# kakaobrain/hqtransformer

Hardware: NVIDIA B200
Metric: images_per_sec_sampled_256x256 (higher is better)
Workload: dtype bf16

## Files before the change

### hqtransformer_b200/_lib.py

```python
from __future__ import annotations

import ctypes as C
import os

PKG_DIR = os.path.dirname(os.path.abspath(__file__))
LIB_PATH = os.path.join(PKG_DIR, "libhqgraft.so")
ABI_VERSION = 8

HQ_OK = 0
HQ_COND_CLS, HQ_COND_TXT, HQ_COND_UNCOND = 0, 1, 2
HQ_PREC_BF16, HQ_PREC_FP32 = 0, 1
HQ_F32, HQ_BF16, HQ_F16 = 0, 1, 2
HQ_MODEL = {"parallel": 0, "top2bot": 1, "bidirectional": 2}
HQ_EMB = {"transformer1": 0, "reduce": 1}
HQ_POS = {"1d": 0, "2d": 1}


class HQConfig(C.Structure):
    _fields_ = [(n, C.c_int32) for n in (
        "embed_dim", "n_heads", "n_layers", "n_layers_depth", "vocab_top", "vocab_bot", "vocab_txt", "n_classes",
        "ctx_len_img", "ctx_len_txt", "cond_kind", "precision", "max_seq_len", "use_cuda_graph", "use_pdl", "use_chain", "model_type", "embedding_kind",
        "position_kind", "code_levels", "vocab_mid", "fuse_head_sampler")]


class HQSamplingParams(C.Structure):
    _fields_ = [("top_k_top", C.c_int32), ("top_k_bot", C.c_int32),
                ("top_p_top", C.c_float), ("top_p_bot", C.c_float),
                ("temperature_top", C.c_float), ("temperature_bot", C.c_float),
                ("seed", C.c_uint64), ("row_offset", C.c_uint64),
                ("top_k_mid", C.c_int32), ("top_p_mid", C.c_float), ("temperature_mid", C.c_float), ("reserved", C.c_int32)]


class HQRunArgs(C.Structure):
    _fields_ = [("batch", C.c_int32), ("seq_len", C.c_int32), ("pos_begin", C.c_int32), ("pos_end", C.c_int32),
                ("cond", C.c_void_p), ("sos", C.c_void_p), ("given_top", C.c_void_p), ("given_bot", C.c_void_p),
                ("codes_top", C.c_void_p), ("codes_bot", C.c_void_p), ("logits", C.c_void_p),
                ("sampling", HQSamplingParams), ("codes_mid", C.c_void_p), ("given_mid", C.c_void_p),
                ("shared_prefix", C.c_int32), ("reserved", C.c_int32)]


class HQS1Config(C.Structure):
    _fields_ = [("embed_dim", C.c_int32), ("n_embed", C.c_int32), ("z_channels", C.c_int32), ("resolution", C.c_int32),
                ("ch", C.c_int32), ("ch_mult", C.c_int32 * 8), ("n_levels", C.c_int32), ("num_res_blocks", C.c_int32),
                ("attn_resolution", C.c_int32), ("out_ch", C.c_int32)]


PROTOTYPES = {
    "hq_abi_version": (C.c_int, []),
    "hq_last_error": (C.c_char_p, [C.c_void_p]),
    "hq_create": (C.c_int, [C.POINTER(HQConfig), C.c_int, C.c_int, C.POINTER(C.c_void_p)]),
    "hq_destroy": (C.c_int, [C.c_void_p]),
    "hq_reserve_batch": (C.c_int, [C.c_void_p, C.c_int]),
    "hq_max_batch": (C.c_int, [C.c_void_p]),
    "hq_load_param": (C.c_int, [C.c_void_p, C.c_char_p, C.c_void_p, C.c_int, C.POINTER(C.c_int64), C.c_int, C.c_int]),
    "hq_params_complete": (C.c_int, [C.c_void_p]),
    "hq_run": (C.c_int, [C.c_void_p, C.POINTER(HQRunArgs), C.c_void_p]),
    "hq_run_host": (C.c_int, [C.c_void_p, C.POINTER(HQRunArgs)]),
    "hq_last_launch_count": (C.c_int64, [C.c_void_p]),
    "hq_device_bytes": (C.c_size_t, [C.c_void_p]),
    "hq_chain_launch_count": (C.c_int64, [C.c_void_p]),
    "hq_debug_gemm": (C.c_int, [C.c_int, C.c_void_p, C.c_void_p, C.c_void_p, C.c_int, C.c_int, C.c_int, C.c_int,
                             C.c_void_p]),
    "hq_debug_philox": (C.c_int, [C.c_uint64, C.POINTER(C.c_uint32), C.POINTER(C.c_uint32)]),
    "hq_debug_sample": (C.c_int, [C.c_void_p, C.c_int, C.c_int, C.c_float, C.c_int, C.c_float, C.c_uint64, C.c_uint64,
                                  C.c_int, C.c_int, C.c_void_p, C.c_void_p, C.c_void_p]),
    "hq_debug_attention": (C.c_int, [C.c_int, C.c_void_p, C.c_void_p, C.c_void_p, C.c_void_p, C.c_int, C.c_int, C.c_int,
                                     C.c_int, C.c_int, C.c_void_p]),
    "hq_debug_attention_phases": (C.c_int, [C.c_void_p, C.c_int, C.c_int, C.c_int, C.POINTER(C.c_uint64), C.c_int,
                                            C.POINTER(C.c_int), C.c_void_p]),
    "hq_debug_chain_phases": (C.c_int, [C.c_void_p, C.POINTER(HQRunArgs), C.c_void_p, C.c_int, C.c_int, C.POINTER(C.c_uint64),
                                        C.c_int, C.POINTER(C.c_int)]),
    "hq_bench_attention": (C.c_int, [C.c_void_p, C.c_int, C.c_int, C.c_int, C.POINTER(C.c_float), C.c_void_p]),
    "hq_trace_run": (C.c_int, [C.c_void_p, C.POINTER(HQRunArgs), C.c_void_p, C.POINTER(C.c_uint64), C.c_char_p, C.c_int,
                               C.POINTER(C.c_int)]),
    "hq_debug_gemm_phases": (C.c_int, [C.c_void_p, C.POINTER(HQRunArgs), C.c_void_p, C.c_int, C.POINTER(C.c_uint64), C.c_int,
                                       C.POINTER(C.c_uint64), C.c_char_p, C.c_int, C.POINTER(C.c_int)]),
    "hq_bench_gemm_shape": (C.c_int, [C.c_int, C.c_int, C.c_int, C.c_int, C.c_int, C.c_int, C.c_int, C.POINTER(C.c_float),
                                      C.POINTER(C.c_float), C.c_void_p]),
    "hq_bench_gemm": (C.c_int, [C.c_void_p, C.c_int, C.c_int, C.c_int, C.POINTER(C.c_float), C.c_void_p]),
    "hq_s1_create": (C.c_int, [C.POINTER(HQS1Config), C.c_int, C.c_int, C.POINTER(C.c_void_p)]),
    "hq_s1_destroy": (C.c_int, [C.c_void_p]),
    "hq_s1_last_error": (C.c_char_p, [C.c_void_p]),
    "hq_s1_device_bytes": (C.c_size_t, [C.c_void_p]),
    "hq_s1_load_param": (C.c_int, [C.c_void_p, C.c_char_p, C.c_void_p, C.c_int, C.POINTER(C.c_int64), C.c_int, C.c_int]),
    "hq_s1_params_complete": (C.c_int, [C.c_void_p]),
    "hq_s1_decode_codes": (C.c_int, [C.c_void_p, C.c_void_p, C.c_void_p, C.c_void_p, C.c_int, C.c_void_p]),
    "hq_s1_last_conv_flops": (C.c_double, [C.c_void_p]),
}

_lib = None


class HQError(RuntimeError):
    pass


def load() -> C.CDLL:
    global _lib
    if _lib is not None:
        return _lib
    if not os.path.isfile(LIB_PATH):
        raise ImportError(
            f"{LIB_PATH} is missing: build it with `python hqtransformer_b200/build.py` "
            "(hqtransformer_b200 has no CPU or PyTorch fallback path)")
    path = LIB_PATH
    if os.environ.get("HQ_DEBUG", "0") not in ("", "0") and os.environ.get("HQGRAFT_LIB"):
        path = os.environ["HQGRAFT_LIB"]
    lib = C.CDLL(path)
    for name, (res, args) in PROTOTYPES.items():
        fn = getattr(lib, name)
        fn.restype = res
        fn.argtypes = args
    got = lib.hq_abi_version()
    if got != ABI_VERSION:
        raise ImportError(f"libhqgraft.so ABI version {got} != binding version {ABI_VERSION}: rebuild the library")
    _lib = lib
    return lib


def check(rc: int, ctx=None, what: str = "") -> None:
    if rc != HQ_OK:
        msg = load().hq_last_error(ctx)
        raise HQError(f"{what or 'libhqgraft'} failed (status {rc}): {msg.decode() if msg else '?'}")


def check_s1(rc: int, ctx, lib, what: str = "") -> None:
    if rc != HQ_OK:
        msg = lib.hq_s1_last_error(ctx)
        raise HQError(f"{what or 'libhqgraft stage 1'} failed (status {rc}): {msg.decode() if msg else '?'}")
```

### hqtransformer_b200/csrc/engine.cu

```cuda
#include <cuda.h>
#include <cuda_runtime.h>

#include <cstdarg>
#include <cstdio>
#include <cstdlib>
#include <algorithm>
#include <cstring>
#include <map>
#include <string>
#include <tuple>
#include <vector>

#include "../../include/hqgraft.h"
#include "common.cuh"
#include "gemm.cuh"
#include "kernels.cuh"
#include "chain.cuh"

using namespace hq;

static thread_local std::string g_last_error;

struct hq_ctx;
static void set_err(hq_ctx* ctx, const char* fmt, ...);
// ... 63 lines not shown
  int bench_splits = 0;
  int force_bn = 0;
  int no_chain = 0;
  int chain_min_batch = 0;
  int chain_no_l2pf = 0;
  int gemm_ks1 = 0;
  int bn_m256 = 0;
};

static int env_int(const char* name) {
  const char* v = getenv(name);
  return v ? atoi(v) : 0;
}
static DebugSwitches read_debug_switches() {
  DebugSwitches d;
  const char* on = getenv("HQ_DEBUG");
  if (on == nullptr || atoi(on) == 0) return d;
  if (const char* a = getenv("HQ_ABLATE")) d.ablate = a;
  d.attn_groups = env_int("HQ_ATTN_GROUPS");
  d.attn_no_prefetch = getenv("HQ_ATTN_NO_PREFETCH") != nullptr;
  d.attn_sleep = env_int("HQ_ATTN_SLEEP");
  d.attn_scalar = getenv("HQ_ATTN_SCALAR") != nullptr;
  d.attm_stages = env_int("HQ_ATTM_STAGES");
  d.attm_per_sm = env_int("HQ_ATTM_PER_SM");
  d.attn_generic = getenv("HQ_ATTN_GENERIC") != nullptr;
  d.attn_fewkeys_old = getenv("HQ_ATTN_FEWKEYS_OLD") != nullptr;
  d.max_splitk = env_int("HQ_MAX_SPLITK");
  d.no_splitk = getenv("HQ_NO_SPLITK") != nullptr;
  d.force_splitk = env_int("HQ_FORCE_SPLITK");
  d.trace_pdl = getenv("HQ_TRACE_PDL") != nullptr;
  d.bench_splits = env_int("HQ_BENCH_SPLITS");
  d.no_chain = getenv("HQ_NO_CHAIN") != nullptr;
  d.chain_min_batch = env_int("HQ_CHAIN_MIN_BATCH");
  d.chain_no_l2pf = getenv("HQ_CHAIN_NO_L2PF") != nullptr;
  d.gemm_ks1 = getenv("HQ_GEMM_KS1") != nullptr;
  d.bn_m256 = env_int("HQ_BN_M256");
  return d;
}

struct GraphKey {
  int B, S, p0, p1, forced_top, forced_bot, sos_override, tracing;
  bool operator<(const GraphKey& o) const {
    return std::tie(B, S, p0, p1, forced_top, forced_bot, sos_override, tracing) <
           std::tie(o.B, o.S, o.p0, o.p1, o.forced_top, o.forced_bot, o.sos_override, o.tracing);
  }
};

struct hq_ctx {
  hq_config cfg;
  int device = 0, max_batch = 0;
  bool bf16 = true;
  int D = 0, nh = 0, L = 0, Ld = 0, Vt = 0, Vb = 0, Vmax = 0, T0 = 1, Tc = 0, Smax = 0;
  size_t wsize = 2;
  std::string err;
  std::vector<void*> allocs;
  std::vector<void*> act_allocs;
  bool alloc_act = false;
  size_t device_bytes = 0, act_bytes = 0;
  std::map<std::string, ParamSlot> params;
  PFN_encodeTiled encode = nullptr;

  std::vector<BlockW> blocks, depths;
  Weight head_top, head_bot;
  float *sos_table = nullptr, *sos_depth = nullptr;
  float *E_top = nullptr, *E_bot = nullptr, *P_emb = nullptr, *P_top = nullptr;
  float *E_txt = nullptr, *P_txt = nullptr;
  float *E_top_depth = nullptr, *P_depth = nullptr;
  float *E_bot_depth = nullptr;
  float *P_top_h = nullptr, *P_top_w = nullptr;
  int Hpos = 0;
  int depth_rows = 4;
  int levels = 2, n_stack = 5, Vm = 0;
  float *E_mid = nullptr, *E_mid_depth = nullptr, *P_depth2 = nullptr, *lnm_g = nullptr, *lnm_b = nullptr;
  Weight head_mid;
  int64_t* codes_mid = nullptr;
  float *lnf_g = nullptr, *lnf_b = nullptr, *lnt_g = nullptr, *lnt_b = nullptr, *lnb_g = nullptr, *lnb_b = nullptr;

  ABuf h, att, mlp;
  void* q = nullptr;
  float *x = nullptr, *yd = nullptr, *logits = nullptr;
  float2* samp_part = nullptr;
  float* splitk_ws = nullptr;
  unsigned int* att_sched = nullptr;
  CUtensorMap kmap, vmap;
  bool kv_maps = false;
  int num_sms = 0;
  int ws_rows = 0;
  void *kc = nullptr, *vc = nullptr, *kd = nullptr, *vd = nullptr;
  int64_t *cond = nullptr, *codes_top = nullptr, *codes_bot = nullptr;
  float* sos_override = nullptr;
  hq_sampling_params* d_sp = nullptr;

  cudaStream_t own_stream = nullptr;
  struct GraphEntry { cudaGraphExec_t exec; int64_t launches; uint64_t stamp; };
  static constexpr size_t kMaxGraphs = 96;
  std::map<GraphKey, GraphEntry> graphs;
  int64_t launches = 0;
  int64_t last_launches = 0;
  cudaError_t launch_err = cudaSuccess;
  bool use_pdl = false;
  bool tracing = false;
  int trace_cap = 0;
  std::vector<std::string> trace_tags;
  bool full_dependency_next = false;
  std::string tag_suffix;
  DebugSwitches dbg = read_debug_switches();
  uint64_t graph_clock = 0;

  bool chain_ok = false;
  int chain_grid = 0;
  CUtensorMap* d_maps = nullptr;
  ChainOp* d_ops = nullptr;
  int ops_cap = 0, ops_used = 0;
  std::map<std::string, int> chain_index;
  unsigned long long* d_chain_bar = nullptr;
  unsigned long long chain_epoch = 0;
  enum { CHAIN_OFF = 0, CHAIN_PLAN = 1, CHAIN_RUN = 2 };
  int chain_mode = CHAIN_OFF;
  bool recording = false;
  std::vector<ChainOp> rec;
  std::vector<std::string> rec_tags;
  int rec_flags = 0;
  const char* gemm_tag_override = nullptr;
  ChainRt chain_rt;
  std::vector<char> trace_chain_cont;
  int64_t chain_launches = 0, chain_ops = 0;
  int chain_launches_run = 0;
  int phase_launch = -1, phase_op = -1;
};

static void set_err(hq_ctx* ctx, const char* fmt, ...) {
  char buf[2048];
  va_list ap;
  va_start(ap, fmt);
  vsnprintf(buf, sizeof(buf), fmt, ap);
  va_end(ap);
  g_last_error = buf;
  if (ctx) ctx->err = buf;
}

static int dev_alloc(hq_ctx* ctx, void** p, size_t bytes) {
  bytes = (bytes + 255) & ~static_cast<size_t>(255);
  HQ_CUDA(ctx, cudaMalloc(p, bytes));
  HQ_CUDA(ctx, cudaMemset(*p, 0, bytes));
  if (ctx->alloc_act) {
    ctx->act_allocs.push_back(*p);
    ctx->act_bytes += bytes;
  } else {
    ctx->allocs.push_back(*p);
    ctx->device_bytes += bytes;
  }
  return HQ_OK;
}

static int make_map(hq_ctx* ctx, CUtensorMap* m, void* base, uint64_t rows, uint64_t cols, uint32_t box_rows) {
  cuuint64_t dims[2] = {cols, rows};
  cuuint64_t strides[1] = {cols * 2};
  cuuint32_t box[2] = {64, box_rows};
  cuuint32_t estr[2] = {1, 1};
  CUresult r = ctx->encode(m, CU_TENSOR_MAP_DATA_TYPE_BFLOAT16, 2, base, dims, strides, box, estr,
                           CU_TENSOR_MAP_INTERLEAVE_NONE, CU_TENSOR_MAP_SWIZZLE_128B, CU_TENSOR_MAP_L2_PROMOTION_L2_256B,
                           CU_TENSOR_MAP_FLOAT_OOB_FILL_NONE);
  if (r != CUDA_SUCCESS) {
    set_err(ctx, "cuTensorMapEncodeTiled failed (%d) rows=%llu cols=%llu", static_cast<int>(r),
            static_cast<unsigned long long>(rows), static_cast<unsigned long long>(cols));
    return HQ_ERR_CUDA;
  }
  return HQ_OK;
}

static int make_map3(hq_ctx* ctx, CUtensorMap* m, void* base, uint64_t rows, uint64_t cols, uint32_t box_rows, uint32_t ks) {
  cuuint64_t dims[3] = {64, rows, cols / 64};
  cuuint64_t strides[2] = {cols * 2, 128};
  cuuint32_t box[3] = {64, box_rows, ks};
  cuuint32_t estr[3] = {1, 1, 1};
  CUresult r = ctx->encode(m, CU_TENSOR_MAP_DATA_TYPE_BFLOAT16, 3, base, dims, strides, box, estr,
                           CU_TENSOR_MAP_INTERLEAVE_NONE, CU_TENSOR_MAP_SWIZZLE_128B, CU_TENSOR_MAP_L2_PROMOTION_L2_256B,
                           CU_TENSOR_MAP_FLOAT_OOB_FILL_NONE);
  if (r != CUDA_SUCCESS) {
    set_err(ctx, "cuTensorMapEncodeTiled (3-D k-block view) failed (%d) rows=%llu cols=%llu box_rows=%u", static_cast<int>(r),
            static_cast<unsigned long long>(rows), static_cast<unsigned long long>(cols), box_rows);
    return HQ_ERR_CUDA;
  }
  return HQ_OK;
}

static int make_pair_maps(hq_ctx* ctx, PairMaps* pm, void* base, uint64_t rows, uint64_t cols) {
  memset(pm, 0, sizeof(*pm));
  pm->have3 = cols >= 128;
  for (int i = 0; i < 6; ++i) {
    if (static_cast<uint64_t>(PairMaps::width(i)) > rows) continue;
    int rc = make_map(ctx, &pm->m[i], base, rows, cols, static_cast<uint32_t>(PairMaps::width(i) / 2));
    if (rc) return rc;
    if (pm->have3 && (rc = make_map3(ctx, &pm->m3[i], base, rows, cols, static_cast<uint32_t>(PairMaps::width(i) / 2), 2))) return rc;
  }
  return HQ_OK;
}

static int make_kv_map(hq_ctx* ctx, CUtensorMap* m, const void* base, int n_heads, uint64_t rows, int hpc) {
  cuuint64_t dims[3] = {64, static_cast<cuuint64_t>(n_heads), rows};
  cuuint64_t strides[2] = {128, static_cast<cuuint64_t>(n_heads) * 128};
  cuuint32_t box[3] = {64, static_cast<cuuint32_t>(hpc), 8};
  cuuint32_t estr[3] = {1, 1, 1};
  CUresult r = ctx->encode(m, CU_TENSOR_MAP_DATA_TYPE_BFLOAT16, 3, const_cast<void*>(base), dims, strides, box, estr,
                           CU_TENSOR_MAP_INTERLEAVE_NONE, CU_TENSOR_MAP_SWIZZLE_128B, CU_TENSOR_MAP_L2_PROMOTION_L2_256B,
                           CU_TENSOR_MAP_FLOAT_OOB_FILL_NONE);
  if (r != CUDA_SUCCESS) {
    set_err(ctx, "cuTensorMapEncodeTiled (KV cache) failed (%d) heads=%d rows=%llu hpc=%d", static_cast<int>(r), n_heads,
            static_cast<unsigned long long>(rows), hpc);
    return HQ_ERR_CUDA;
  }
  return HQ_OK;
}

static int alloc_weight(hq_ctx* ctx, Weight* w, int N, int K) {
  w->N = N;
  w->K = K;
  int rc = dev_alloc(ctx, &w->ptr, static_cast<size_t>(N) * K * ctx->wsize);
  if (rc) return rc;
  if (ctx->bf16) {
    if ((rc = make_map(ctx, &w->map, w->ptr, N, K, 64))) return rc;
    return make_pair_maps(ctx, &w->mapp, w->ptr, N, K);
  }
  return HQ_OK;
}
static int alloc_abuf(hq_ctx* ctx, ABuf* a, int rows, int K) {
  a->rows = (rows + 127) / 128 * 128;
  a->K = K;
  int rc = dev_alloc(ctx, &a->ptr, static_cast<size_t>(a->rows) * K * ctx->wsize);
  if (rc) return rc;
  if (ctx->bf16) {
    if ((rc = make_map(ctx, &a->map, a->ptr, a->rows, K, 128))) return rc;
    a->have3 = K >= 128;
    if (a->have3) return make_map3(ctx, &a->map3, a->ptr, a->rows, K, 128, 2);
  }
  return HQ_OK;
}
static int alloc_f32(hq_ctx* ctx, float** p, size_t n) { return dev_alloc(ctx, reinterpret_cast<void**>(p), n * 4); }

static void reg(hq_ctx* ctx, const std::string& name, void* dst, int is_weight, std::vector<int64_t> shape,
                bool ignored = false) {
  ParamSlot s;
  s.dst = dst;
  s.dst_is_weight = is_weight;
  s.shape = shape;
  s.ignored = ignored;
  ctx->params[name] = s;
}

static int build_block(hq_ctx* ctx, BlockW* b, const std::string& prefix) {
  const int D = ctx->D;
  int rc;
  if ((rc = alloc_weight(ctx, &b->qkv, 3 * D, D))) return rc;
  if ((rc = alloc_weight(ctx, &b->proj, D, D))) return rc;
  if ((rc = alloc_weight(ctx, &b->fc1, 4 * D, D))) return rc;
  if ((rc = alloc_weight(ctx, &b->fc2, D, 4 * D))) return rc;
  if ((rc = alloc_f32(ctx, &b->bqkv, 3 * D))) return rc;
  if ((rc = alloc_f32(ctx, &b->bproj, D))) return rc;
  if ((rc = alloc_f32(ctx, &b->b1, 4 * D))) return rc;
  if ((rc = alloc_f32(ctx, &b->b2, D))) return rc;
  float** lns[4] = {&b->ln1g, &b->ln1b, &b->ln2g, &b->ln2b};
  for (auto p : lns)
    if ((rc = alloc_f32(ctx, p, D))) return rc;
  const size_t wsz = ctx->wsize;
  char* wq = static_cast<char*>(b->qkv.ptr);
  reg(ctx, prefix + ".attn.query.weight", wq, 1, {D, D});
  reg(ctx, prefix + ".attn.key.weight", wq + static_cast<size_t>(D) * D * wsz, 1, {D, D});
  reg(ctx, prefix + ".attn.value.weight", wq + static_cast<size_t>(2) * D * D * wsz, 1, {D, D});
  reg(ctx, prefix + ".attn.query.bias", b->bqkv, 0, {D});
  reg(ctx, prefix + ".attn.key.bias", b->bqkv + D, 0, {D});
  reg(ctx, prefix + ".attn.value.bias", b->bqkv + 2 * D, 0, {D});
  reg(ctx, prefix + ".attn.proj.weight", b->proj.ptr, 1, {D, D});
  reg(ctx, prefix + ".attn.proj.bias", b->bproj, 0, {D});
  reg(ctx, prefix + ".mlp.0.weight", b->fc1.ptr, 1, {4 * D, D});
  reg(ctx, prefix + ".mlp.0.bias", b->b1, 0, {4 * D});
  reg(ctx, prefix + ".mlp.2.weight", b->fc2.ptr, 1, {D, 4 * D});
  reg(ctx, prefix + ".mlp.2.bias", b->b2, 0, {D});
  reg(ctx, prefix + ".ln1.weight", b->ln1g, 0, {D});
  reg(ctx, prefix + ".ln1.bias", b->ln1b, 0, {D});
  reg(ctx, prefix + ".ln2.weight", b->ln2g, 0, {D});
  reg(ctx, prefix + ".ln2.bias", b->ln2b, 0, {D});
  return HQ_OK;
}

template <typename K>
static int set_smem(hq_ctx* ctx, K kernel, int bytes) {
  HQ_CUDA(ctx, cudaFuncSetAttribute(kernel, cudaFuncAttributeMaxDynamicSharedMemorySize, bytes));
  return HQ_OK;
}

static int set_gemm_attrs(hq_ctx* ctx) {
  int rc;
#define HQ_SET(BN, EPI) \
// ... 61 lines not shown
extern "C" int hq_destroy(hq_ctx* ctx) {
  if (!ctx) return HQ_OK;
  cudaSetDevice(ctx->device);
  cudaDeviceSynchronize();
  free_activations(ctx);
  for (void* p : ctx->allocs) cudaFree(p);
  if (ctx->own_stream) cudaStreamDestroy(ctx->own_stream);
  delete ctx;
  return HQ_OK;
}

static void free_activations(hq_ctx* ctx) {
  for (auto& kv : ctx->graphs) cudaGraphExecDestroy(kv.second.exec);
  ctx->graphs.clear();
  for (void* p : ctx->act_allocs) cudaFree(p);
  ctx->act_allocs.clear();
  ctx->act_bytes = 0;
  ctx->d_maps = nullptr;
  ctx->chain_index.clear();
  ctx->ops_used = 0;
}

static int reserve_alloc(hq_ctx* ctx, int max_batch);

static int reserve_impl(hq_ctx* ctx, int max_batch) {
  const int rc = reserve_alloc(ctx, max_batch);
  if (rc != HQ_OK) {
    const std::string why = ctx->err;
    cudaGetLastError();
    free_activations(ctx);
    ctx->max_batch = 0;
    ctx->ws_rows = 0;
    ctx->kv_maps = false;
    ctx->h = ABuf(); ctx->att = ABuf(); ctx->mlp = ABuf();
    ctx->q = nullptr; ctx->x = nullptr; ctx->yd = nullptr; ctx->logits = nullptr; ctx->samp_part = nullptr; ctx->splitk_ws = nullptr;
    ctx->kc = ctx->vc = ctx->kd = ctx->vd = nullptr;
    ctx->cond = ctx->codes_top = ctx->codes_bot = ctx->codes_mid = nullptr;
    ctx->sos_override = nullptr;
    ctx->d_sp = nullptr;
    set_err(ctx, "hq_reserve_batch(%d) failed, the ctx holds no batch state until a reserve succeeds: %s", max_batch,
            why.c_str());
  }
  return rc;
}

static int reserve_alloc(hq_ctx* ctx, int max_batch) {
  int rc;
  if (max_batch < 1) {
    set_err(ctx, "max_batch must be >= 1");
    return HQ_ERR_INVALID;
  }
  HQ_CUDA(ctx, cudaSetDevice(ctx->device));
  HQ_CUDA(ctx, cudaDeviceSynchronize());
  free_activations(ctx);
  ctx->max_batch = max_batch;
  ctx->alloc_act = true;
  struct Guard { hq_ctx* c; ~Guard() { c->alloc_act = false; } } guard{ctx};
  const int D = ctx->D;
  const int B = max_batch;
  const int Mx = B * ctx->T0;
  const int Mmax = (ctx->depth_rows * B > Mx) ? ctx->depth_rows * B : Mx;
  if ((rc = alloc_abuf(ctx, &ctx->h, Mmax, D))) return rc;
  if ((rc = alloc_abuf(ctx, &ctx->att, Mmax, D))) return rc;
  if ((rc = alloc_abuf(ctx, &ctx->mlp, Mmax, 4 * D))) return rc;
  if ((rc = dev_alloc(ctx, &ctx->q, static_cast<size_t>(Mmax) * D * ctx->wsize))) return rc;
  if ((rc = alloc_f32(ctx, &ctx->x, static_cast<size_t>(Mx) * D))) return rc;
  if ((rc = alloc_f32(ctx, &ctx->yd, static_cast<size_t>(ctx->depth_rows) * B * D))) return rc;
  if ((rc = alloc_f32(ctx, &ctx->logits, static_cast<size_t>(ctx->depth_rows < 4 ? 4 : ctx->depth_rows) * B * ctx->Vmax))) return rc;
  {
    float* sp2 = nullptr;
    if ((rc = alloc_f32(ctx, &sp2, static_cast<size_t>(ctx->depth_rows < 4 ? 4 : ctx->depth_rows) * B * ((ctx->Vmax + 31) / 32) * 2))) return rc;
    ctx->samp_part = reinterpret_cast<float2*>(sp2);
  }
  ctx->ws_rows = Mmax;
  if (ctx->bf16 && (rc = alloc_f32(ctx, &ctx->splitk_ws, static_cast<size_t>(LN_MAXFOLD) * Mmax * D))) return rc;
  const size_t kvn = static_cast<size_t>(ctx->L) * B * ctx->Tc * D * ctx->wsize;
  if ((rc = dev_alloc(ctx, &ctx->kc, kvn))) return rc;
  if ((rc = dev_alloc(ctx, &ctx->vc, kvn))) return rc;
  ctx->kv_maps = false;
  if (ctx->bf16) {
    const int groups = attn_groups(ctx, ctx->nh);
    if (groups > 0) {
      const uint64_t rows = static_cast<uint64_t>(ctx->L) * B * ctx->Tc;
      if ((rc = make_kv_map(ctx, &ctx->kmap, ctx->kc, ctx->nh, rows, ctx->nh / groups))) return rc;
      if ((rc = make_kv_map(ctx, &ctx->vmap, ctx->vc, ctx->nh, rows, ctx->nh / groups))) return rc;
      ctx->kv_maps = true;
    }
  }
  const size_t kdn = static_cast<size_t>(ctx->Ld) * B * ctx->n_stack * D * ctx->wsize;
  if ((rc = dev_alloc(ctx, &ctx->kd, kdn))) return rc;
  if ((rc = dev_alloc(ctx, &ctx->vd, kdn))) return rc;
  if ((rc = dev_alloc(ctx, reinterpret_cast<void**>(&ctx->cond), static_cast<size_t>(B) * ctx->T0 * 8))) return rc;
  if ((rc = dev_alloc(ctx, reinterpret_cast<void**>(&ctx->codes_top), static_cast<size_t>(B) * ctx->Smax * 8))) return rc;
  if ((rc = dev_alloc(ctx, reinterpret_cast<void**>(&ctx->codes_bot),
                      static_cast<size_t>(B) * ctx->Smax * 8 * (ctx->levels == 3 ? 16 : 4)))) return rc;
  if (ctx->levels == 3 &&
      (rc = dev_alloc(ctx, reinterpret_cast<void**>(&ctx->codes_mid), static_cast<size_t>(B) * ctx->Smax * 32))) return rc;
  if ((rc = alloc_f32(ctx, &ctx->sos_override, static_cast<size_t>(Mx) * D))) return rc;
  if ((rc = dev_alloc(ctx, reinterpret_cast<void**>(&ctx->d_sp), sizeof(hq_sampling_params)))) return rc;
  if (ctx->bf16) {
    std::vector<CUtensorMap> table;
    ABuf* abufs[3] = {&ctx->h, &ctx->att, &ctx->mlp};
    for (ABuf* a : abufs) {
      a->map_idx = static_cast<int>(table.size());
      table.push_back(a->map);
    }
    auto add_w = [&](Weight& w) {
      w.map_idx = static_cast<int>(table.size());
      for (int i = 0; i < 6; ++i) table.push_back(w.mapp.m[i]);
    };
    for (auto& b : ctx->blocks) { add_w(b.qkv); add_w(b.proj); add_w(b.fc1); add_w(b.fc2); }
    for (auto& b : ctx->depths) { add_w(b.qkv); add_w(b.proj); add_w(b.fc1); add_w(b.fc2); }
    add_w(ctx->head_top);
    add_w(ctx->head_bot);
    if (ctx->levels == 3) add_w(ctx->head_mid);
    if ((rc = dev_alloc(ctx, reinterpret_cast<void**>(&ctx->d_maps), table.size() * sizeof(CUtensorMap)))) return rc;
    HQ_CUDA(ctx, cudaMemcpy(ctx->d_maps, table.data(), table.size() * sizeof(CUtensorMap), cudaMemcpyHostToDevice));
  }
  return HQ_OK;
}

static int create_impl(hq_ctx* ctx, const hq_config* cfg, int device, int max_batch) {
  int rc;
  if ((rc = check_device(ctx, device))) return rc;
  HQ_CUDA(ctx, cudaSetDevice(device));
  ctx->cfg = *cfg;
  ctx->device = device;
  ctx->max_batch = max_batch;
  ctx->bf16 = cfg->precision == HQ_PREC_BF16;
  ctx->use_pdl = cfg->use_pdl != 0;
  ctx->wsize = ctx->bf16 ? 2 : 4;
  const int D = ctx->D = cfg->embed_dim;
  ctx->nh = cfg->n_heads;
  ctx->L = cfg->n_layers;
  ctx->Ld = cfg->n_layers_depth;
  ctx->Vt = cfg->vocab_top;
  ctx->Vb = cfg->vocab_bot;
  ctx->Vmax = ctx->Vt > ctx->Vb ? ctx->Vt : ctx->Vb;
  ctx->levels = cfg->code_levels == 3 ? 3 : 2;
  if (cfg->code_levels != 0 && cfg->code_levels != 2 && cfg->code_levels != 3) {
    set_err(ctx, "code_levels must be 2 or 3 (got %d)", cfg->code_levels);
    return HQ_ERR_INVALID;
  }
  if (ctx->levels == 3) {
    ctx->Vm = cfg->vocab_mid;
    ctx->n_stack = 21;
    if (ctx->Vm > ctx->Vmax) ctx->Vmax = ctx->Vm;
    if (ctx->Vm < 64 || ctx->Vm % 64 != 0 || cfg->cond_kind == HQ_COND_TXT || cfg->model_type != HQ_MODEL_PARALLEL ||
        cfg->embedding_kind != HQ_EMB_TRANSFORMER1 || cfg->position_kind != HQ_POS_1D) {
      set_err(ctx, "code_levels == 3: the 'parallel-add' HQTransformer with class / unconditional sos, 'transformer1' embedding and "
                   "1-D positions is implemented (vocab_mid a multiple of 64)");
      return HQ_ERR_UNSUPPORTED;
    }
  }
  ctx->Smax = cfg->max_seq_len;
  const bool txt = cfg->cond_kind == HQ_COND_TXT;
  ctx->T0 = txt ? cfg->ctx_len_txt : 1;
  ctx->Tc = ctx->T0 + ctx->Smax - 1;
  if (max_batch < 1 || D < 64 || D % 64 != 0 || ctx->nh * 64 != D) {
    set_err(ctx, "unsupported shape: embed_dim=%d n_heads=%d (head size must be 64), max_batch=%d", D, ctx->nh, max_batch);
    return HQ_ERR_UNSUPPORTED;
  }
  if (ctx->Vt % 64 != 0 || ctx->Vb % 64 != 0 || ctx->Vmax > 32768) {
    set_err(ctx, "unsupported vocabulary sizes %d / %d (multiples of 64, <= 32768)", ctx->Vt, ctx->Vb);
    return HQ_ERR_UNSUPPORTED;
  }
  if (ctx->Tc > ATT_MAX_KEYS || ctx->Smax < 1 || ctx->Smax > cfg->ctx_len_img) {
    set_err(ctx, "unsupported lengths: max_seq_len=%d ctx_len_img=%d ctx_len_txt=%d (cache length %d > %d)", ctx->Smax,
// ... 505 lines not shown
  size_t stride = 0;
  const float* bias = nullptr;
};

template <typename AT>
static void layernorm_act(hq_ctx* ctx, cudaStream_t st, float* x, const float* g, const float* b, AT* out, int rows,
                          Fold* fold = nullptr) {
  Fold f = fold ? *fold : Fold();
  if (ctx->recording) {
    ChainOp* op = chain_push(ctx, CH_OP_LN, "layernorm");
    op->flags = sizeof(AT) == 4 ? CH_F_OUT_F32 : 0;
    op->x = x; op->gamma = g; op->beta = b; op->add = nullptr; op->out = out;
    op->rows = rows; op->in_mul = 1; op->in_off = 0; op->D = ctx->D;
    op->fold = f.partial; op->n_fold = f.n; op->fold_stride = f.stride; op->fold_bias = f.bias;
    if (fold) *fold = Fold();
    return;
  }
  auto kern = f.n > 3 ? layernorm_kernel<AT, LN_MAXFOLD> : layernorm_kernel<AT, 3>;
  launch_k(ctx, st, "layernorm", kern, dim3(rows), dim3(LN_THREADS), 0, x, g, b, nullptr, out, rows,
           ctx->D, 1, 0, f.partial, f.n, f.stride, f.bias, 1, 1);
  if (fold) *fold = Fold();
}

template <typename OutT>
static void layernorm_rows(hq_ctx* ctx, cudaStream_t st, const char* tag, float* x, const float* g, const float* b,
                           const float* add, OutT* out, int rows, int in_group, int in_mul, int in_off, int out_mul,
                           const Fold& f) {
  auto kern = f.n > 3 ? layernorm_kernel<OutT, LN_MAXFOLD> : layernorm_kernel<OutT, 3>;
  launch_k(ctx, st, tag, kern, dim3(rows), dim3(LN_THREADS), 0, x, g, b, add, out, rows, ctx->D, in_mul, in_off, f.partial,
           f.n, f.stride, f.bias, in_group, out_mul);
}

static bool attn_prefetch_ok(const hq_ctx* ctx) { return !ctx->dbg.attn_no_prefetch; }

static int attn_sleep_ns(const hq_ctx* ctx) { return ctx->dbg.attn_sleep; }

template <typename AT>
static bool attn_decode_plan(const hq_ctx* ctx, int* CH, int* hpc, int* groups, size_t* smem) {
  const int g = attn_groups(ctx, ctx->nh);
  if (g <= 0) return false;
  *groups = g;
  *hpc = ctx->nh / g;
  const int row_bytes = *hpc * 64 * static_cast<int>(sizeof(AT));
  int ch = (6144 / row_bytes) / 4 * 4;
  if (ch < 4) ch = 4;
  if (ch > 16) ch = 16;
  *CH = ch;
  *smem = static_cast<size_t>(ATTD_STAGES) * ch * row_bytes + static_cast<size_t>(*hpc) * ATT_MAX_KEYS * 4 +
          2 * ATTD_STAGES * 8 + 128;
  return *smem <= 64 * 1024;
}

static bool attn_mma_plan(const hq_ctx* ctx, int groups, int hpc, int n_items, int* stages, size_t* smem, int* grid) {
  if (ctx->dbg.attn_scalar || !ctx->bf16 || ctx->num_sms <= 0 || !ctx->kv_maps) return false;
  const size_t stage = static_cast<size_t>(2 * ATTM_CH) * hpc * 128;
  int st = 2;
  if (ctx->dbg.attm_stages) st = ctx->dbg.attm_stages;
  if (st < 2) st = 2;
  if (st > ATTM_MAXSTAGES) st = ATTM_MAXSTAGES;
  const size_t bytes = 1024  + st * stage + 2 * static_cast<size_t>(hpc) * 128 +
                       static_cast<size_t>(hpc) * 64 * 4 + (2 * ATTM_MAXSTAGES + 4) * 8 + 16;
  if (bytes > 112 * 1024) return false;
  int per_sm = static_cast<int>((227 * 1024) / (bytes + 1024));
  const int by_threads = 2048 / ((hpc + 1) * 32);
  if (per_sm > by_threads) per_sm = by_threads;
  const int by_regs = 65536 / ((hpc + 1) * 32 * 72);
  if (by_regs >= 1 && per_sm > by_regs) per_sm = by_regs;
  if (ctx->dbg.attm_per_sm > 0 && ctx->dbg.attm_per_sm < per_sm) per_sm = ctx->dbg.attm_per_sm;
  if (per_sm < 1) per_sm = 1;
  (void)groups;
  *stages = st;
  *smem = bytes;
  const int cap = ctx->num_sms * per_sm;
  *grid = n_items < cap ? n_items : cap;
  return true;
}

template <typename AT>
static void launch_attn_mma(hq_ctx*, cudaStream_t, const AT*, const AT*, AT*, int, int, int, int, int, int, int, size_t) {}
template <>
void launch_attn_mma<bf16>(hq_ctx* ctx, cudaStream_t st, const bf16* q, const bf16* K, bf16* out, int t_stride, int n_keys,
                           int hpc, int groups, int n_items, int stages, int grid, size_t smem) {
  const int row_base = static_cast<int>((K - static_cast<const bf16*>(ctx->kc)) / ctx->D);
  launch_k(ctx, st, "attention_decode", attention_decode_mma_kernel, dim3(grid), dim3((hpc + 1) * 32), smem, ctx->kmap, ctx->vmap,
           row_base, q, out, ctx->D, t_stride, n_keys, hpc, groups, n_items, attn_prefetch_ok(ctx) ? stages : -stages,
           ctx->att_sched);
}

template <typename AT>
static void attention(hq_ctx* ctx, cudaStream_t st, const AT* q, const AT* K, const AT* V, AT* out, int M, int Tq,
                      int t_stride, int kbase, int causal) {
  int CH = 0, hpc = 0, groups = 0;
  size_t smem = 0;
  if (ctx->recording && sizeof(AT) == 2 && !causal && kbase <= ATT_DEPTH_KEYS && Tq == 4) {
    ChainOp* op = chain_push(ctx, CH_OP_ATTN4, "attention_depth4");
    op->q = reinterpret_cast<const bf16*>(q); op->kc = reinterpret_cast<const bf16*>(K);
    op->vc = reinterpret_cast<const bf16*>(V); op->att = reinterpret_cast<bf16*>(out);
    op->B = M / 4; op->n_heads = ctx->nh; op->D = ctx->D; op->t_stride = t_stride; op->n_keys = kbase;
    return;
  }
  const bool resume = ctx->recording;
  if (resume) chain_flush(ctx, st);
  struct Resume { hq_ctx* c; bool on; ~Resume() { c->recording = on; } } resume_guard{ctx, resume};
  ctx->recording = false;
  if (Tq == 1 && !causal && !ctx->dbg.attn_generic && attn_decode_plan<AT>(ctx, &CH, &hpc, &groups, &smem)) {
    if (ctx->tracing) ctx->tag_suffix = ":t" + std::to_string(kbase) + ":B" + std::to_string(M);
    int stages = 0, grid = 0;
    size_t smem2 = 0;
    const ptrdiff_t koff = reinterpret_cast<const char*>(K) - static_cast<const char*>(ctx->kc);
    const ptrdiff_t kv_bytes = static_cast<ptrdiff_t>(ctx->L) * ctx->max_batch * ctx->Tc * ctx->D * static_cast<ptrdiff_t>(ctx->wsize);
    const bool in_cache = ctx->kc != nullptr && koff >= 0 && (koff < kv_bytes || ctx->L == 0) &&
                          koff == reinterpret_cast<const char*>(V) - static_cast<const char*>(ctx->vc);
    if (sizeof(AT) == 2 && in_cache && attn_mma_plan(ctx, groups, hpc, M * groups, &stages, &smem2, &grid)) {
      launch_attn_mma<AT>(ctx, st, q, K, out, t_stride, kbase, hpc, groups, M * groups, stages, grid, smem2);
      return;
    }
    launch_k(ctx, st, "attention_decode", attention_decode_kernel<AT>, dim3(M * groups), dim3((hpc + 1) * 32), smem, q, K, V,
             out, ctx->D, t_stride, kbase, CH, hpc, groups, attn_prefetch_ok(ctx) ? attn_sleep_ns(ctx) : -1);
    return;
  }
  const int items = M * ctx->nh;
  if (!causal && kbase <= ATT_DEPTH_KEYS && Tq == 4 && !ctx->dbg.attn_fewkeys_old) {
    const int warps = (M / 4) * ctx->nh;
    launch_k(ctx, st, "attention_depth4", attention_depth4_kernel<AT>, dim3((warps + ATT_WARPS - 1) / ATT_WARPS),
             dim3(ATT_WARPS * 32), 0, q, K, V, out, M / 4, ctx->nh, ctx->D, t_stride, kbase);
    return;
  }
  if (!causal && kbase <= 8) {
    launch_k(ctx, st, "attention_fewkeys", attention_fewkeys_kernel<AT>, dim3((items + ATT_WARPS - 1) / ATT_WARPS),
             dim3(ATT_WARPS * 32), 0, q, K, V, out, M, ctx->nh, ctx->D, Tq, t_stride, kbase);
    return;
  }
  launch_k(ctx, st, "attention_generic", attention_kernel<AT>, dim3((items + ATT_WARPS - 1) / ATT_WARPS),
           dim3(ATT_WARPS * 32), 0, q, K, V, out, M, ctx->nh, ctx->D, Tq, t_stride, kbase, causal);
}

static void launch_sample(hq_ctx* ctx, cudaStream_t st, const SampleArgs& a) {
  if (a.V <= 256 * SMP_IPT) launch_k(ctx, st, "sample", sample_kernel<256>, dim3(a.R), dim3(256), 0, a);
  else launch_k(ctx, st, "sample", sample_kernel<1024>, dim3(a.R), dim3(1024), 0, a);
}

static void gemm_fc2_split(hq_ctx* ctx, cudaStream_t st, const ABuf& A, const Weight& W, int M, int N, int K, int splits,
                           int bn, bf16*) {
  EpiParams<bf16> e;
  memset(&e, 0, sizeof(e));
  e.outf = ctx->splitk_ws; e.ldo = N; e.split_stride = static_cast<size_t>(ctx->ws_rows) * N;
  ctx->gemm_tag_override = "gemm_resid";
  gemm_bf16<EPI_F32>(ctx, st, A.map, A.have3 ? &A.map3 : nullptr, W.map, W.mapp, 0, M, N, K, e, splits, bn, A.map_idx, W.map_idx);
}
static void gemm_fc2_split(hq_ctx*, cudaStream_t, const ABuf&, const Weight&, int, int, int, int, int, float*) {}

struct Fc2Plan { int bn, splits; };

static int resid_splits(const hq_ctx* ctx, int N, int K, int rows_per_image) {
  static const int cand[6] = {256, 192, 128, 96, 64, 32};
  const int kb = K / 64;
  const int max_splits = ctx->dbg.max_splitk > 0 ? ctx->dbg.max_splitk : (kb % 3 == 0 ? 3 : LN_MAXFOLD);
  int best = 1;
  double best_cost = 1e30;
  for (int bn : cand) {
    if (N % bn != 0) continue;
    for (int s = 1; s <= max_splits && s <= LN_MAXFOLD; ++s) {
      if (kb % s != 0) continue;
      const double cost = pair_gemm_cost(256 * (rows_per_image < 1 ? 1 : rows_per_image), N, K, bn, s);
      if (cost < best_cost) {
        best_cost = cost;
        best = s;
      }
    }
  }
  return best;
}

static Fc2Plan pick_resid_plan(const hq_ctx* ctx, int M, int N, int K, int rows_per_image) {
  Fc2Plan best{0, 1};
  if (!ctx->bf16 || N % 64 != 0 || K % 64 != 0 || ctx->dbg.no_splitk) return best;
  static const int cand[6] = {256, 192, 128, 96, 64, 32};
  const int kb = K / 64;
  int s = resid_splits(ctx, N, K, rows_per_image);
  {
    const int v = ctx->dbg.force_splitk;
    if (v >= 1 && v <= LN_MAXFOLD && kb % v == 0) s = v;
  }
  best.splits = s;
  if (M <= 128) return best;
  double best_cost = 1e30;
  for (int bn : cand) {
    if (N % bn != 0) continue;
    const double cost = pair_gemm_cost(M, N, K, bn, s);
    if (cost < best_cost) {
      best_cost = cost;
      best.bn = bn;
    }
  }
  return best;
}

template <typename AT>
static void gemm_resid(hq_ctx* ctx, cudaStream_t st, const ABuf& A, const Weight& W, const float* bias, float* x, int M,
                       int N, int K, int rows_per_image, Fold* fold) {
  const Fc2Plan plan = pick_resid_plan(ctx, M, N, K, rows_per_image);
  if (plan.splits > 1 && M <= ctx->ws_rows) {
    gemm_fc2_split(ctx, st, A, W, M, N, K, plan.splits, plan.bn, static_cast<AT*>(nullptr));
    fold->partial = ctx->splitk_ws;
    fold->n = plan.splits;
    fold->stride = static_cast<size_t>(ctx->ws_rows) * N;
    fold->bias = bias;
    return;
  }
  EpiParams<AT> e;
  memset(&e, 0, sizeof(e));
  e.bias = bias; e.x = x;
  gemm_any<EPI_RESID>(ctx, st, A, W, 0, M, N, K, e);
}

template <typename AT>
static void run_block(hq_ctx* ctx, cudaStream_t st, const BlockW& w, float* x, int M, int mode, AT* kdst, AT* vdst,
                      int rpb, int t_stride, int t0, int n_keys_base, int causal, Fold* fold) {
  const int D = ctx->D;
  AT* h = static_cast<AT*>(ctx->h.ptr);
  AT* att = static_cast<AT*>(ctx->att.ptr);
  AT* mlp = static_cast<AT*>(ctx->mlp.ptr);
  AT* q = static_cast<AT*>(ctx->q);
  layernorm_act<AT>(ctx, st, x, w.ln1g, w.ln1b, h, M, fold);
  EpiParams<AT> ep;
  memset(&ep, 0, sizeof(ep));
  ep.q = q; ep.kdst = kdst; ep.vdst = vdst; ep.D = D; ep.rpb = rpb; ep.t_stride = t_stride; ep.t0 = t0;
  if (mode == 1) {
    ep.bias = w.bqkv + D; ep.sec0 = 1; ep.vdup = att;
    gemm_any<EPI_QKV>(ctx, st, ctx->h, w.qkv, D, M, 2 * D, D, ep);
  } else {
    ep.bias = w.bqkv; ep.sec0 = 0; ep.vdup = nullptr;
    if (mode == 0) ctx->rec_flags = CH_F_T0_RT;
    gemm_any<EPI_QKV>(ctx, st, ctx->h, w.qkv, 0, M, 3 * D, D, ep);
    ctx->rec_flags = 0;
    attention<AT>(ctx, st, q, kdst, vdst, att, M, rpb, t_stride, n_keys_base, causal);
  }
  gemm_resid<AT>(ctx, st, ctx->att, w.proj, w.bproj, x, M, D, D, rpb, fold);
  layernorm_act<AT>(ctx, st, x, w.ln2g, w.ln2b, h, M, fold);
  EpiParams<AT> eg;
  memset(&eg, 0, sizeof(eg));
  eg.bias = w.b1; eg.out = mlp;
  gemm_any<EPI_GELU>(ctx, st, ctx->h, w.fc1, 0, M, 4 * D, D, eg);
  gemm_resid<AT>(ctx, st, ctx->mlp, w.fc2, w.b2, x, M, D, 4 * D, rpb, fold);
}

struct RunFlags {
  int forced_top, forced_bot, sos_override, forced_mid;
  int shared_prefix;
  int fuse_mask;
  float* logits_out;
};

template <typename AT>
static bool head_gemm(hq_ctx* ctx, cudaStream_t st, const Weight& w, int rows, int V, const SampleArgs& sa, const RunFlags& f) {
  const bool fuse = sizeof(AT) == 2 && !ctx->recording && ((f.fuse_mask >> sa.filt_sel) & 1) && !sa.forced &&
                    sa.logits_out == nullptr && V % 32 == 0;
  EpiParams<AT> e;
  memset(&e, 0, sizeof(e));
  if (fuse) {
    e.sp = sa.sp; e.samp_part = ctx->samp_part; e.temp_sel = sa.temp_sel; e.rows_per_b = sa.rows_per_b; e.slot0 = sa.slot0;
    e.pos = sa.pos;
    ctx->gemm_tag_override = "gemm_head_sample";
    gemm_any<EPI_SAMPLE>(ctx, st, ctx->h, w, 0, rows, V, ctx->D, e);
  } else {
    e.outf = ctx->logits; e.ldo = ctx->Vmax;
    gemm_any<EPI_F32>(ctx, st, ctx->h, w, 0, rows, V, ctx->D, e);
  }
  return fuse;
}

static void draw(hq_ctx* ctx, cudaStream_t st, const SampleArgs& sa, bool fused) {
  if (fused)
    launch_k(ctx, st, "sample_finalize", sample_finalize_kernel, dim3((sa.R + SMPF_WARPS - 1) / SMPF_WARPS), dim3(SMPF_WARPS * 32),
             0, sa, static_cast<const float2*>(ctx->samp_part), sa.V / 32);
  else if (!(sa.forced && sa.logits_out == nullptr))
    launch_sample(ctx, st, sa);
}

template <typename AT>
static void run_position(hq_ctx* ctx, cudaStream_t st, int B, int S, int pos, const RunFlags& f) {
  const int D = ctx->D, T0 = ctx->T0, Tc = ctx->Tc;
  const bool txt = ctx->cfg.cond_kind == HQ_COND_TXT;
  const bool prefill = txt && pos == 0;
  const bool shared = prefill && f.shared_prefix && B > 1;
  const int Bp = shared ? 1 : B;
  const int M = prefill ? Bp * T0 : B;
  AT* kc = static_cast<AT*>(ctx->kc);
  AT* vc = static_cast<AT*>(ctx->vc);
  AT* kd = static_cast<AT*>(ctx->kd);
  AT* vd = static_cast<AT*>(ctx->vd);
  AT* h = static_cast<AT*>(ctx->h.ptr);
  const size_t lstride = static_cast<size_t>(ctx->max_batch) * Tc * D;
  const size_t dstride = static_cast<size_t>(ctx->max_batch) * 5 * D;

  const int eb = (D / 4 + 31) / 32 * 32 > 1024 ? 1024 : (D / 4 + 31) / 32 * 32;
  Fold fold_x, fold_y;
  ctx->full_dependency_next = true;
  if (prefill) {
    launch_k(ctx, st, "embed_txt", embed_txt_kernel, dim3(M), dim3(eb), 0, ctx->x, f.sos_override ? ctx->sos_override : nullptr,
             ctx->cond, ctx->E_txt, ctx->P_txt, T0, D);
  } else {
    EmbedArgs ea;
    ea.x = ctx->x; ea.sos_table = ctx->sos_table; ea.sos_override = f.sos_override ? ctx->sos_override : nullptr;
    ea.cond = ctx->cond; ea.E_top = ctx->E_top; ea.E_bot = ctx->E_bot; ea.P_top = ctx->P_top; ea.P_emb = ctx->P_emb;
    ea.codes_top = ctx->codes_top; ea.codes_bot = ctx->codes_bot; ea.D = D; ea.S = S; ea.pos = pos;
    ea.cond_kind = ctx->cfg.cond_kind;
    ea.emb_kind = ctx->cfg.embedding_kind; ea.P_top_h = ctx->P_top_h; ea.P_top_w = ctx->P_top_w; ea.Hpos = ctx->Hpos;
    launch_k(ctx, st, "embed", embed_kernel, dim3(B), dim3(eb), 0, ea);
  }

  const int tok = (pos == 0) ? 0 : T0 + pos - 1;
  const bool chain = sizeof(AT) == 2 && !prefill && chain_enabled(ctx, B);
  if (chain) chain_begin(ctx, tok, pos, S);
  for (int l = 0; l < ctx->L; ++l) {
    if (prefill) run_block<AT>(ctx, st, ctx->blocks[l], ctx->x, M, 0, kc + l * lstride, vc + l * lstride, T0, Tc, 0, 0, 1, &fold_x);
    else run_block<AT>(ctx, st, ctx->blocks[l], ctx->x, M, 0, kc + l * lstride, vc + l * lstride, 1, Tc, tok, tok + 1, 0, &fold_x);
  }
  if (ctx->recording) {
    ChainOp* op = chain_push(ctx, CH_OP_LN, "layernorm_f");
    op->flags = CH_F_OUT_F32;
    op->x = ctx->x; op->gamma = ctx->lnf_g; op->beta = ctx->lnf_b; op->add = ctx->sos_depth; op->out = ctx->yd;
    op->rows = B; op->in_mul = 1; op->in_off = 0; op->D = D;
    op->fold = fold_x.partial; op->n_fold = fold_x.n; op->fold_stride = fold_x.stride; op->fold_bias = fold_x.bias;
  } else {
    launch_k(ctx, st, "layernorm_f", fold_x.n > 3 ? layernorm_kernel<float, LN_MAXFOLD> : layernorm_kernel<float, 3>, dim3(B),
             dim3(LN_THREADS), 0, ctx->x, ctx->lnf_g, ctx->lnf_b,
             ctx->sos_depth, ctx->yd, prefill ? Bp : B, D, prefill ? T0 : 1, prefill ? T0 - 1 : 0, fold_x.partial, fold_x.n, fold_x.stride,
             fold_x.bias, 1, ctx->cfg.model_type == HQ_MODEL_BIDIRECTIONAL ? 5 : 1);
  }
  fold_x = Fold();
  if (shared)
    launch_k(ctx, st, "broadcast_prefix", broadcast_prefix_kernel<AT>, dim3(T0, ctx->L, B - 1), dim3(256), 0, kc, vc, ctx->yd,
             ctx->max_batch, Tc, D);

  SampleArgs sa;
  memset(&sa, 0, sizeof(sa));
  sa.logits = ctx->logits; sa.ldl = ctx->Vmax; sa.V = ctx->Vt; sa.R = B; sa.rows_per_b = 1; sa.slot0 = 0;
  sa.sp = ctx->d_sp; sa.pos = pos; sa.S = S; sa.dst_codes = ctx->codes_top; sa.dst_w = 1; sa.n_slots = ctx->n_stack;
  sa.forced = f.forced_top; sa.logits_out = f.logits_out; sa.Vmax = ctx->Vmax;
  sa.temp_sel = 0; sa.filt_sel = 0; sa.bot_slot = -1;
  if (ctx->cfg.model_type == HQ_MODEL_TOP2BOT) {
    for (int c = 0; c < 5; ++c) {
      if (c >= 1) {
        const float* E = c == 1 ? ctx->E_top_depth : ctx->E_bot_depth;
        const int64_t* codes = c == 1 ? ctx->codes_top + pos : ctx->codes_bot + static_cast<size_t>(pos) * 4 + (c - 2);
        launch_k(ctx, st, "embed_depth_seq", embed_depth_seq_kernel, dim3(B), dim3(eb), 0, ctx->yd, E,
                 static_cast<const float*>(ctx->P_depth + static_cast<size_t>(c - 1) * D), codes, c == 1 ? S : 4 * S, D);
      }
      for (int l = 0; l < ctx->Ld; ++l)
        run_block<AT>(ctx, st, ctx->depths[l], ctx->yd, B, 0, kd + l * dstride, vd + l * dstride, 1, 5, c, c + 1, 0, &fold_y);
      layernorm_act<AT>(ctx, st, ctx->yd, c == 0 ? ctx->lnt_g : ctx->lnb_g, c == 0 ? ctx->lnt_b : ctx->lnb_b, h, B, &fold_y);
      sa.V = c == 0 ? ctx->Vt : ctx->Vb; sa.slot0 = c; sa.bot_slot = c - 1;
      sa.dst_codes = c == 0 ? ctx->codes_top : ctx->codes_bot; sa.dst_w = c == 0 ? 1 : 4;
      sa.temp_sel = sa.filt_sel = c == 0 ? 0 : 1;
      sa.forced = c == 0 ? f.forced_top : f.forced_bot;
      draw(ctx, st, sa, head_gemm<AT>(ctx, st, c == 0 ? ctx->head_top : ctx->head_bot, B, sa.V, sa, f));
    }
    return;
  }
  if (ctx->cfg.model_type == HQ_MODEL_BIDIRECTIONAL) {
    launch_k(ctx, st, "depth_pos_rows", depth_pos_rows_kernel, dim3(B), dim3(eb), 0, ctx->yd, static_cast<const float*>(ctx->P_depth), D);
    for (int l = 0; l < ctx->Ld; ++l)
      run_block<AT>(ctx, st, ctx->depths[l], ctx->yd, 5 * B, 2, kd + l * dstride, vd + l * dstride, 5, 5, 0, 5, 0, &fold_y);
    layernorm_rows<AT>(ctx, st, "layernorm", ctx->yd, ctx->lnt_g, ctx->lnt_b, nullptr, h, B, 1, 5, 0, 1, fold_y);
    sa.temp_sel = 0; sa.filt_sel = 1;
    draw(ctx, st, sa, head_gemm<AT>(ctx, st, ctx->head_top, B, ctx->Vt, sa, f));
    layernorm_rows<AT>(ctx, st, "layernorm", ctx->yd, ctx->lnb_g, ctx->lnb_b, nullptr, h, 4 * B, 4, 5, 1, 1, fold_y);
    fold_y = Fold();
    sa.V = ctx->Vb; sa.R = 4 * B; sa.rows_per_b = 4; sa.slot0 = 1; sa.forced = f.forced_bot;
    sa.dst_codes = ctx->codes_bot; sa.dst_w = 4;
    draw(ctx, st, sa, head_gemm<AT>(ctx, st, ctx->head_bot, 4 * B, ctx->Vb, sa, f));
    return;
  }

  for (int l = 0; l < ctx->Ld; ++l)
    run_block<AT>(ctx, st, ctx->depths[l], ctx->yd, B, 1, kd + l * dstride, vd + l * dstride, 1, 5, 0, 1, 0, &fold_y);
  layernorm_act<AT>(ctx, st, ctx->yd, ctx->lnt_g, ctx->lnt_b, h, B, &fold_y);
  {
    const bool fused = head_gemm<AT>(ctx, st, ctx->head_top, B, ctx->Vt, sa, f);
    if (chain) chain_end(ctx, st);
    draw(ctx, st, sa, fused);
  }

  if (chain) {
    chain_begin(ctx, tok, pos, S);
    ChainOp* op = chain_push(ctx, CH_OP_EMBED_DEPTH, "embed_depth");
    op->y = ctx->yd; op->E = ctx->E_top_depth; op->P = ctx->P_depth; op->codes_top = ctx->codes_top; op->B = B; op->D = D;
  } else {
    launch_k(ctx, st, "embed_depth", embed_depth_kernel, dim3(B), dim3(eb), 0, ctx->yd, ctx->E_top_depth, ctx->P_depth,
             ctx->codes_top, S, pos, D);
  }
  for (int l = 0; l < ctx->Ld; ++l)
    run_block<AT>(ctx, st, ctx->depths[l], ctx->yd, 4 * B, 2, kd + l * dstride, vd + l * dstride, 4, 5, 1, 5, 0, &fold_y);
  layernorm_act<AT>(ctx, st, ctx->yd, ctx->lnb_g, ctx->lnb_b, h, 4 * B, &fold_y);
  sa.V = ctx->Vb; sa.R = 4 * B; sa.rows_per_b = 4; sa.slot0 = 1; sa.forced = f.forced_bot;
  sa.temp_sel = 1; sa.filt_sel = 1; sa.dst_codes = ctx->codes_bot; sa.dst_w = 4;
  {
    const bool fused = head_gemm<AT>(ctx, st, ctx->head_bot, 4 * B, ctx->Vb, sa, f);
    if (chain) chain_end(ctx, st);
    draw(ctx, st, sa, fused);
  }
}

template <typename AT>
static void run_position3(hq_ctx* ctx, cudaStream_t st, int B, int S, int pos, const RunFlags& f) {
  const int D = ctx->D, Tc = ctx->Tc;
  AT* kc = static_cast<AT*>(ctx->kc);
  AT* vc = static_cast<AT*>(ctx->vc);
  AT* kd = static_cast<AT*>(ctx->kd);
  AT* vd = static_cast<AT*>(ctx->vd);
  AT* h = static_cast<AT*>(ctx->h.ptr);
  const size_t lstride = static_cast<size_t>(ctx->max_batch) * Tc * D;
  const size_t dstride = static_cast<size_t>(ctx->max_batch) * 21 * D;
  const int eb = (D / 4 + 31) / 32 * 32 > 1024 ? 1024 : (D / 4 + 31) / 32 * 32;
  Fold fold_x, fold_y;
  ctx->full_dependency_next = true;
  Embed3Args ea;
  ea.x = ctx->x; ea.sos_table = ctx->sos_table; ea.sos_override = f.sos_override ? ctx->sos_override : nullptr;
  ea.cond = ctx->cond; ea.E0 = ctx->E_top; ea.E1 = ctx->E_mid; ea.E2 = ctx->E_bot; ea.P_top = ctx->P_top; ea.P_emb = ctx->P_emb;
  ea.codes_top = ctx->codes_top; ea.codes_mid = ctx->codes_mid; ea.codes_bot = ctx->codes_bot;
  ea.D = D; ea.S = S; ea.pos = pos; ea.cond_kind = ctx->cfg.cond_kind;
  launch_k(ctx, st, "embed", embed3_kernel, dim3(B), dim3(eb), 0, ea);
  const int tok = pos;
  for (int l = 0; l < ctx->L; ++l)
    run_block<AT>(ctx, st, ctx->blocks[l], ctx->x, B, 0, kc + l * lstride, vc + l * lstride, 1, Tc, tok, tok + 1, 0, &fold_x);
  launch_k(ctx, st, "layernorm_f", fold_x.n > 3 ? layernorm_kernel<float, LN_MAXFOLD> : layernorm_kernel<float, 3>, dim3(B),
           dim3(LN_THREADS), 0, ctx->x, ctx->lnf_g, ctx->lnf_b, ctx->sos_depth, ctx->yd, B, D, 1, 0, fold_x.partial, fold_x.n,
           fold_x.stride, fold_x.bias, 1, 1);
  fold_x = Fold();

  SampleArgs sa;
  memset(&sa, 0, sizeof(sa));
  sa.logits = ctx->logits; sa.ldl = ctx->Vmax; sa.sp = ctx->d_sp; sa.pos = pos; sa.S = S; sa.n_slots = 21;
  sa.logits_out = f.logits_out; sa.Vmax = ctx->Vmax; sa.bot_slot = -1;
  for (int l = 0; l < ctx->Ld; ++l)
    run_block<AT>(ctx, st, ctx->depths[l], ctx->yd, B, 1, kd + l * dstride, vd + l * dstride, 1, 21, 0, 1, 0, &fold_y);
  layernorm_act<AT>(ctx, st, ctx->yd, ctx->lnt_g, ctx->lnt_b, h, B, &fold_y);
  sa.V = ctx->Vt; sa.R = B; sa.rows_per_b = 1; sa.slot0 = 0; sa.temp_sel = sa.filt_sel = 0;
  sa.dst_codes = ctx->codes_top; sa.dst_w = 1; sa.forced = f.forced_top;
  draw(ctx, st, sa, head_gemm<AT>(ctx, st, ctx->head_top, B, ctx->Vt, sa, f));
  launch_k(ctx, st, "embed_depth", embed_depth_kernel, dim3(B), dim3(eb), 0, ctx->yd, ctx->E_top_depth, ctx->P_depth,
           ctx->codes_top, S, pos, D);
  for (int l = 0; l < ctx->Ld; ++l)
    run_block<AT>(ctx, st, ctx->depths[l], ctx->yd, 4 * B, 2, kd + l * dstride, vd + l * dstride, 4, 21, 1, 5, 0, &fold_y);
  layernorm_act<AT>(ctx, st, ctx->yd, ctx->lnm_g, ctx->lnm_b, h, 4 * B, &fold_y);
  sa.V = ctx->Vm; sa.R = 4 * B; sa.rows_per_b = 4; sa.slot0 = 1; sa.temp_sel = sa.filt_sel = 2;
  sa.dst_codes = ctx->codes_mid; sa.dst_w = 4; sa.forced = f.forced_mid;
  draw(ctx, st, sa, head_gemm<AT>(ctx, st, ctx->head_mid, 4 * B, ctx->Vm, sa, f));
  launch_k(ctx, st, "embed_depth2", embed_depth2_kernel, dim3(B), dim3(eb), 0, ctx->yd, ctx->E_mid_depth, ctx->E_top_depth,
           ctx->P_depth2, ctx->codes_top, ctx->codes_mid, S, pos, D);
  for (int l = 0; l < ctx->Ld; ++l)
    run_block<AT>(ctx, st, ctx->depths[l], ctx->yd, 16 * B, 2, kd + l * dstride, vd + l * dstride, 16, 21, 5, 21, 0, &fold_y);
  layernorm_act<AT>(ctx, st, ctx->yd, ctx->lnb_g, ctx->lnb_b, h, 16 * B, &fold_y);
  sa.V = ctx->Vb; sa.R = 16 * B; sa.rows_per_b = 16; sa.slot0 = 5; sa.temp_sel = sa.filt_sel = 1;
  sa.dst_codes = ctx->codes_bot; sa.dst_w = 16; sa.forced = f.forced_bot;
  draw(ctx, st, sa, head_gemm<AT>(ctx, st, ctx->head_bot, 16 * B, ctx->Vb, sa, f));
}

static void run_range(hq_ctx* ctx, cudaStream_t st, int B, int S, int p0, int p1, const RunFlags& f) {
  if (ctx->levels == 3) {
    for (int pos = p0; pos < p1; ++pos) {
      if (ctx->bf16) run_position3<bf16>(ctx, st, B, S, pos, f);
      else run_position3<float>(ctx, st, B, S, pos, f);
    }
    return;
  }
  for (int pos = p0; pos < p1; ++pos) {
    if (ctx->bf16) run_position<bf16>(ctx, st, B, S, pos, f);
    else run_position<float>(ctx, st, B, S, pos, f);
  }
}

static int validate_run(hq_ctx* ctx, const hq_run_args* a) {
  if (!ctx || !a) return HQ_ERR_INVALID;
  int rc = hq_params_complete(ctx);
  if (rc) return rc;
// ... 122 lines not shown
        if (graph) cudaGraphDestroy(graph);
        return HQ_ERR_CUDA;
      }
      cudaGraphExec_t exec = nullptr;
      cudaError_t ie = cudaGraphInstantiate(&exec, graph, 0);
      cudaGraphDestroy(graph);
      if (ie != cudaSuccess) {
        set_err(ctx, "cudaGraphInstantiate failed: %s", cudaGetErrorString(ie));
        return HQ_ERR_CUDA;
      }
      if (ctx->graphs.size() >= hq_ctx::kMaxGraphs) {
        auto victim = ctx->graphs.begin();
        for (auto g = ctx->graphs.begin(); g != ctx->graphs.end(); ++g)
          if (g->second.stamp < victim->second.stamp) victim = g;
        HQ_CUDA(ctx, cudaStreamSynchronize(st));
        cudaGraphExecDestroy(victim->second.exec);
        ctx->graphs.erase(victim);
      }
      it = ctx->graphs.emplace(key, hq_ctx::GraphEntry{exec, ctx->launches, 0}).first;
    }
    it->second.stamp = ++ctx->graph_clock;
    HQ_CUDA(ctx, cudaGraphLaunch(it->second.exec, st));
    ctx->last_launches = it->second.launches;
  } else {
    plan_chains();
    run_range(ctx, st, B, S, a->pos_begin, a->pos_end, f);
    ctx->last_launches = ctx->launches;
    if (ctx->launch_err != cudaSuccess) {
      set_err(ctx, "kernel launch failed: %s", cudaGetErrorString(ctx->launch_err));
      if (dev_logits) cudaFree(dev_logits);
      return HQ_ERR_CUDA;
    }
  }

  HQ_CUDA(ctx, cudaMemcpyAsync(a->codes_top, ctx->codes_top, nt, out_kind, st));
  HQ_CUDA(ctx, cudaMemcpyAsync(a->codes_bot, ctx->codes_bot, nb, out_kind, st));
  if (ctx->levels == 3) HQ_CUDA(ctx, cudaMemcpyAsync(a->codes_mid, ctx->codes_mid, nm, out_kind, st));
  if (dev_logits) {
    HQ_CUDA(ctx, cudaMemcpyAsync(a->logits, dev_logits, nlog, cudaMemcpyDeviceToHost, st));
    HQ_CUDA(ctx, cudaStreamSynchronize(st));
    cudaFree(dev_logits);
  }
  return HQ_OK;
}

extern "C" int hq_run(hq_ctx* ctx, const hq_run_args* args, void* stream) {
  return run_impl(ctx, args, static_cast<cudaStream_t>(stream), cudaMemcpyDeviceToDevice, cudaMemcpyDeviceToDevice);
}

extern "C" int hq_run_host(hq_ctx* ctx, const hq_run_args* args) {
  if (!ctx) return HQ_ERR_INVALID;
  int rc = run_impl(ctx, args, ctx->own_stream, cudaMemcpyHostToDevice, cudaMemcpyDeviceToHost);
  if (rc) return rc;
  HQ_CUDA(ctx, cudaStreamSynchronize(ctx->own_stream));
  return HQ_OK;
}

extern "C" int hq_debug_attention(int prec, const void* q, const void* K, const void* V, void* out, int B, int n_heads,
                                  int t_stride, int n_keys, int variant, void* stream) {
  cudaStream_t st = static_cast<cudaStream_t>(stream);
  if (B < 1 || n_heads < 1 || n_keys < 1 || n_keys > t_stride || n_keys > ATT_MAX_KEYS || !q || !K || !V || !out) {
    set_err(nullptr, "hq_debug_attention: bad argument");
    return HQ_ERR_INVALID;
  }
  hq_ctx tmp;
  int dev = 0;
  HQ_CUDA(nullptr, cudaGetDevice(&dev));
  int rc = check_device(&tmp, dev);
  if (rc) return rc;
  tmp.bf16 = prec == HQ_PREC_BF16;
  tmp.D = n_heads * 64;
  tmp.nh = n_heads;
  HQ_CUDA(nullptr, cudaDeviceGetAttribute(&tmp.num_sms, cudaDevAttrMultiProcessorCount, dev));
  if ((rc = set_smem(&tmp, attention_decode_kernel<bf16>, 64 * 1024))) return rc;
  if ((rc = set_smem(&tmp, attention_decode_kernel<float>, 64 * 1024))) return rc;
  if ((rc = set_smem(&tmp, attention_decode_mma_kernel, 112 * 1024))) return rc;
  HQ_CUDA(nullptr, cudaMalloc(reinterpret_cast<void**>(&tmp.att_sched), 16));
  cudaMemsetAsync(tmp.att_sched, 0, 16, st);
  if (tmp.bf16 && variant != 1) {
    const int groups = attn_groups(&tmp, n_heads);
    tmp.kc = const_cast<void*>(K);
    tmp.vc = const_cast<void*>(V);
    if ((rc = get_encode_fn(&tmp, &tmp.encode)) == HQ_OK && groups > 0 &&
        (rc = make_kv_map(&tmp, &tmp.kmap, K, n_heads, static_cast<uint64_t>(B) * t_stride, n_heads / groups)) == HQ_OK &&
        (rc = make_kv_map(&tmp, &tmp.vmap, V, n_heads, static_cast<uint64_t>(B) * t_stride, n_heads / groups)) == HQ_OK)
      tmp.kv_maps = true;
    if (rc) {
      cudaFree(tmp.att_sched);
      set_err(nullptr, "hq_debug_attention: %s", tmp.err.c_str());
      return rc;
    }
  }
  if (variant == 1) tmp.dbg.attn_scalar = 1;
  if (tmp.bf16)
    attention<bf16>(&tmp, st, static_cast<const bf16*>(q), static_cast<const bf16*>(K), static_cast<const bf16*>(V),
                    static_cast<bf16*>(out), B, 1, t_stride, n_keys, 0);
  else
    attention<float>(&tmp, st, static_cast<const float*>(q), static_cast<const float*>(K), static_cast<const float*>(V),
                     static_cast<float*>(out), B, 1, t_stride, n_keys, 0);
  cudaError_t e = cudaStreamSynchronize(st);
  cudaFree(tmp.att_sched);
  if (e == cudaSuccess) e = tmp.launch_err;
  if (e != cudaSuccess) {
    set_err(nullptr, "hq_debug_attention: %s", cudaGetErrorString(e));
    return HQ_ERR_CUDA;
  }
  return HQ_OK;
}

extern "C" int hq_debug_gemm(int prec, const void* A, const void* W, float* C, int M, int N, int K, int tile,
                             void* stream) {
  cudaStream_t st = static_cast<cudaStream_t>(stream);
  hq_ctx tmp;
  if (M < 1 || N < 8 || K < 16) {
    set_err(nullptr, "hq_debug_gemm: bad shape");
    return HQ_ERR_INVALID;
  }
  if (prec == HQ_PREC_FP32) {
    if (K % 16 != 0 || N % 8 != 0) {
      set_err(nullptr, "hq_debug_gemm(fp32): K %% 16 and N %% 8 must be 0");
      return HQ_ERR_INVALID;
    }
    EpiParams<float> e;
    memset(&e, 0, sizeof(e));
    e.outf = C; e.ldo = N;
    gemm_f32<EPI_F32>(&tmp, st, static_cast<const float*>(A), static_cast<const float*>(W), M, N, K, e);
  } else {
    if (K % 64 != 0 || N % 64 != 0) {
      set_err(nullptr, "hq_debug_gemm(bf16): K %% 64 and N %% 64 must be 0");
      return HQ_ERR_INVALID;
    }
    int dev = 0;
    HQ_CUDA(nullptr, cudaGetDevice(&dev));
    int rc = check_device(&tmp, dev);
    if (rc == HQ_OK) rc = get_encode_fn(&tmp, &tmp.encode);
    if (rc == HQ_OK) rc = set_gemm_attrs(&tmp);
    const int Mp = (M + 127) / 128 * 128;
    void* Ap = nullptr;
    if (rc == HQ_OK) {
      HQ_CUDA(nullptr, cudaMalloc(&Ap, static_cast<size_t>(Mp) * K * 2));
      cudaMemsetAsync(Ap, 0, static_cast<size_t>(Mp) * K * 2, st);
      cudaMemcpyAsync(Ap, A, static_cast<size_t>(M) * K * 2, cudaMemcpyDeviceToDevice, st);
    }
    CUtensorMap mA, mA3, mW;
    PairMaps mWp;
    if (rc == HQ_OK) rc = make_map(&tmp, &mA, Ap, Mp, K, 128);
    if (rc == HQ_OK && K >= 128) rc = make_map3(&tmp, &mA3, Ap, Mp, K, 128, 2);
    if (rc == HQ_OK) rc = make_map(&tmp, &mW, const_cast<void*>(W), N, K, 64);
    if (rc == HQ_OK) rc = make_pair_maps(&tmp, &mWp, const_cast<void*>(W), N, K);
    if (rc == HQ_OK) {
      EpiParams<bf16> e;
      memset(&e, 0, sizeof(e));
      e.outf = C; e.ldo = N;
      tmp.dbg.force_bn = tile;
      gemm_bf16<EPI_F32>(&tmp, st, mA, K >= 128 ? &mA3 : nullptr, mW, mWp, 0, M, N, K, e);
    }
    cudaError_t se = cudaStreamSynchronize(st);
    if (Ap) cudaFree(Ap);
    if (rc != HQ_OK) {
      g_last_error = tmp.err;
      return rc;
    }
    if (se != cudaSuccess) {
      set_err(nullptr, "hq_debug_gemm: %s", cudaGetErrorString(se));
      return HQ_ERR_CUDA;
    }
  }
  if (tmp.launch_err != cudaSuccess) {
    set_err(nullptr, "hq_debug_gemm launch failed: %s", cudaGetErrorString(tmp.launch_err));
    return HQ_ERR_CUDA;
  }
  return HQ_OK;
}

extern "C" int hq_debug_philox(uint64_t seed, const uint32_t counter[4], uint32_t out[4]) {
  uint32_t o[4];
  philox4x32_10(static_cast<uint32_t>(seed), static_cast<uint32_t>(seed >> 32), counter[0], counter[1], counter[2],
                counter[3], o);
  for (int i = 0; i < 4; ++i) out[i] = o[i];
  return HQ_OK;
}

extern "C" int hq_debug_sample(const float* logits, int R, int V, float temperature, int top_k, float top_p,
                               uint64_t seed, uint64_t row_offset, int position, int slot, int64_t* out_codes,
                               float* out_probs, void* stream) {
  if (!logits || !out_codes || R < 1 || V < 4 || V % 4 != 0 || V > 32768 || !(temperature > 0.f)) {
    set_err(nullptr, "hq_debug_sample: bad argument");
    return HQ_ERR_INVALID;
  }
  hq_ctx tmp;
  SampleArgs sa;
  memset(&sa, 0, sizeof(sa));
  sa.logits = logits; sa.ldl = V; sa.V = V; sa.R = R; sa.rows_per_b = 1; sa.slot0 = slot; sa.sp = nullptr;
  sa.pos = position; sa.S = 1; sa.flat_out = out_codes; sa.probs_out = out_probs; sa.Vmax = V; sa.n_slots = 5; sa.dst_w = 1;
  sa.temperature = temperature; sa.top_p = top_p; sa.top_k = top_k; sa.seed = seed; sa.row_offset = row_offset;
  sa.bot_slot = -1;
  launch_sample(&tmp, static_cast<cudaStream_t>(stream), sa);
  if (tmp.launch_err != cudaSuccess) {
    set_err(nullptr, "hq_debug_sample launch failed: %s", cudaGetErrorString(tmp.launch_err));
    return HQ_ERR_CUDA;
  }
  return HQ_OK;
}

extern "C" int hq_bench_attention(hq_ctx* ctx, int B, int n_keys, int iters, float* usec, void* stream) {
  if (!ctx || !usec || B < 1 || B > ctx->max_batch || n_keys < 1 || n_keys > ctx->Tc || iters < 1) {
    set_err(ctx, "hq_bench_attention: bad argument");
    return HQ_ERR_INVALID;
  }
  HQ_CUDA(ctx, cudaSetDevice(ctx->device));
  cudaStream_t st = static_cast<cudaStream_t>(stream);
  cudaEvent_t e0, e1;
  HQ_CUDA(ctx, cudaEventCreate(&e0));
  HQ_CUDA(ctx, cudaEventCreate(&e1));
  const size_t lstride = static_cast<size_t>(ctx->max_batch) * ctx->Tc * ctx->D;
  ctx->launch_err = cudaSuccess;
  struct PdlOff { hq_ctx* c; bool saved; PdlOff(hq_ctx* x) : c(x), saved(x->use_pdl) { x->use_pdl = false; } ~PdlOff() { c->use_pdl = saved; } } pdl_off(ctx);
  auto launch = [&](int l) {
    if (ctx->bf16) {
      bf16* kc = static_cast<bf16*>(ctx->kc) + l * lstride;
      bf16* vc = static_cast<bf16*>(ctx->vc) + l * lstride;
      attention<bf16>(ctx, st, static_cast<bf16*>(ctx->q), kc, vc, static_cast<bf16*>(ctx->att.ptr), B, 1, ctx->Tc, n_keys, 0);
    } else {
      float* kc = static_cast<float*>(ctx->kc) + l * lstride;
      float* vc = static_cast<float*>(ctx->vc) + l * lstride;
      attention<float>(ctx, st, static_cast<float*>(ctx->q), kc, vc, static_cast<float*>(ctx->att.ptr), B, 1, ctx->Tc, n_keys, 0);
    }
  };
  for (int i = 0; i < 3; ++i) launch(i % ctx->L);
  HQ_CUDA(ctx, cudaEventRecord(e0, st));
  for (int i = 0; i < iters; ++i) launch(i % ctx->L);
  HQ_CUDA(ctx, cudaEventRecord(e1, st));
  HQ_CUDA(ctx, cudaEventSynchronize(e1));
  float ms = 0.f;
  HQ_CUDA(ctx, cudaEventElapsedTime(&ms, e0, e1));
  cudaEventDestroy(e0);
  cudaEventDestroy(e1);
  if (ctx->launch_err != cudaSuccess) {
    set_err(ctx, "attention launch failed: %s", cudaGetErrorString(ctx->launch_err));
    return HQ_ERR_CUDA;
  }
  *usec = ms * 1000.f / iters;
  return HQ_OK;
}

extern "C" int hq_debug_attention_phases(hq_ctx* ctx, int B, int n_keys, int warm, unsigned long long* out_ns, int max_ctas,
                                         int* n_ctas, void* stream) {
  if (!ctx || !out_ns || !n_ctas || B < 1 || B > ctx->max_batch || n_keys < 1 || n_keys > ctx->Tc || max_ctas < 1) {
    set_err(ctx, "hq_debug_attention_phases: bad argument");
    return HQ_ERR_INVALID;
  }
  HQ_CUDA(ctx, cudaSetDevice(ctx->device));
  cudaStream_t st = static_cast<cudaStream_t>(stream);
  unsigned long long* dev = nullptr;
  const size_t bytes = static_cast<size_t>(max_ctas) * 8 * sizeof(unsigned long long);
  HQ_CUDA(ctx, cudaMalloc(reinterpret_cast<void**>(&dev), bytes));
  HQ_CUDA(ctx, cudaMemsetAsync(dev, 0, bytes, st));
  const size_t lstride = static_cast<size_t>(ctx->max_batch) * ctx->Tc * ctx->D;
  ctx->launch_err = cudaSuccess;
  struct PdlOff { hq_ctx* c; bool saved; PdlOff(hq_ctx* x) : c(x), saved(x->use_pdl) { x->use_pdl = false; } ~PdlOff() { c->use_pdl = saved; } } pdl_off(ctx);
  const int64_t before = ctx->launches;
  auto launch = [&](int l) {
    if (ctx->bf16) {
      bf16* kc = static_cast<bf16*>(ctx->kc) + l * lstride;
      bf16* vc = static_cast<bf16*>(ctx->vc) + l * lstride;
      attention<bf16>(ctx, st, static_cast<bf16*>(ctx->q), kc, vc, static_cast<bf16*>(ctx->att.ptr), B, 1, ctx->Tc, n_keys, 0);
    } else {
      float* kc = static_cast<float*>(ctx->kc) + l * lstride;
      float* vc = static_cast<float*>(ctx->vc) + l * lstride;
      attention<float>(ctx, st, static_cast<float*>(ctx->q), kc, vc, static_cast<float*>(ctx->att.ptr), B, 1, ctx->Tc, n_keys, 0);
    }
  };
  for (int i = 0; i < warm; ++i) launch(i % ctx->L);
  HQ_CUDA(ctx, cudaStreamSynchronize(st));
  HQ_CUDA(ctx, cudaMemcpyToSymbol(g_hq_phase, &dev, sizeof(dev)));
  launch(warm % ctx->L);
  cudaError_t e = cudaStreamSynchronize(st);
  unsigned long long* null_ptr = nullptr;
  cudaMemcpyToSymbol(g_hq_phase, &null_ptr, sizeof(null_ptr));
  (void)before;
  if (e == cudaSuccess) e = ctx->launch_err;
  if (e == cudaSuccess) e = cudaMemcpy(out_ns, dev, bytes, cudaMemcpyDeviceToHost);
// ... 310 lines not shown
```

### hqtransformer_b200/csrc/kernels.cuh

```cuda
#pragma once

#include "common.cuh"
#include "../../include/hqgraft.h"

namespace hq {

struct EmbedArgs {
  float* x;
  const float* sos_table;
  const float* sos_override;
  const int64_t* cond;
  const float* E_top; const float* E_bot; const float* P_top; const float* P_emb;
  const int64_t* codes_top;
  const int64_t* codes_bot;
  int D, S, pos, cond_kind;
  int emb_kind;
  const float* P_top_h;
  const float* P_top_w;
  int Hpos;
};

__global__ void __launch_bounds__(1024) embed_kernel(int trace_id, EmbedArgs a) {
  TraceScope trace_scope(trace_id);
  pdl_launch_dependents();
  pdl_wait();
  const int b = blockIdx.x;
  float4* xo = reinterpret_cast<float4*>(a.x + static_cast<size_t>(b) * a.D);
  const int n4 = a.D / 4;
  if (a.pos == 0) {
    const float* src;
    if (a.sos_override != nullptr) src = a.sos_override + static_cast<size_t>(b) * a.D;
    else if (a.cond_kind == HQ_COND_CLS) src = a.sos_table + static_cast<size_t>(a.cond[b]) * a.D;
    else src = a.sos_table;
    const float4* s4 = reinterpret_cast<const float4*>(src);
    for (int i = threadIdx.x; i < n4; i += blockDim.x) xo[i] = s4[i];
    return;
  }
  const int p = a.pos - 1;
  const int64_t ct = a.codes_top[static_cast<size_t>(b) * a.S + p];
  const int64_t* cbp = a.codes_bot + (static_cast<size_t>(b) * a.S + p) * 4;
  const float4* et = reinterpret_cast<const float4*>(a.E_top + static_cast<size_t>(ct) * a.D);
  const bool pos2d = a.P_top_h != nullptr;
  const float4* pt = reinterpret_cast<const float4*>(pos2d ? a.P_top_h + static_cast<size_t>(p / a.Hpos) * a.D
                                                           : a.P_top + static_cast<size_t>(p) * a.D);
  const float4* pw = pos2d ? reinterpret_cast<const float4*>(a.P_top_w + static_cast<size_t>(p % a.Hpos) * a.D) : nullptr;
  if (a.emb_kind == 1) {
    const int Dq = a.D / 4;
    const float* ebq[4];
#pragma unroll
    for (int j = 0; j < 4; ++j) ebq[j] = a.E_bot + static_cast<size_t>(cbp[j]) * Dq;
    for (int i = threadIdx.x; i < n4; i += blockDim.x) {
      const float4 t = et[i];
      float4 q = pt[i];
      if (pos2d) { const float4 w = pw[i]; q.x += w.x; q.y += w.y; q.z += w.z; q.w += w.w; }
      xo[i] = make_float4((t.x + q.x) + ebq[0][i], (t.y + q.y) + ebq[1][i], (t.z + q.z) + ebq[2][i], (t.w + q.w) + ebq[3][i]);
    }
    return;
  }
  const float4* eb[4];
#pragma unroll
  for (int j = 0; j < 4; ++j) eb[j] = reinterpret_cast<const float4*>(a.E_bot + static_cast<size_t>(cbp[j]) * a.D);
  const float4* pe = reinterpret_cast<const float4*>(a.P_emb);
  for (int i = threadIdx.x; i < n4; i += blockDim.x) {
    float4 t = et[i], q = pt[i], e0 = pe[i];
    if (pos2d) { const float4 w = pw[i]; q.x += w.x; q.y += w.y; q.z += w.z; q.w += w.w; }
    float4 acc;
    acc.x = (t.x + q.x) + e0.x; acc.y = (t.y + q.y) + e0.y; acc.z = (t.z + q.z) + e0.z; acc.w = (t.w + q.w) + e0.w;
#pragma unroll
    for (int j = 0; j < 4; ++j) {
      float4 e = eb[j][i], pj = pe[(j + 1) * n4 + i];
      acc.x += e.x + pj.x; acc.y += e.y + pj.y; acc.z += e.z + pj.z; acc.w += e.w + pj.w;
    }
    acc.x /= 5.0f; acc.y /= 5.0f; acc.z /= 5.0f; acc.w /= 5.0f;
    xo[i] = acc;
  }
}

__global__ void __launch_bounds__(1024)
embed_txt_kernel(int trace_id, float* x, const float* sos_override, const int64_t* ids, const float* E_txt, const float* P_txt,
                 int T, int D) {
  TraceScope trace_scope(trace_id);
  pdl_launch_dependents();
  pdl_wait();
  const int row = blockIdx.x;
  const int t = row % T;
  float4* xo = reinterpret_cast<float4*>(x + static_cast<size_t>(row) * D);
  const int n4 = D / 4;
  if (sos_override != nullptr) {
    const float4* s4 = reinterpret_cast<const float4*>(sos_override + static_cast<size_t>(row) * D);
    for (int i = threadIdx.x; i < n4; i += blockDim.x) xo[i] = s4[i];
    return;
  }
  const float4* e = reinterpret_cast<const float4*>(E_txt + static_cast<size_t>(ids[row]) * D);
  const float4* p = reinterpret_cast<const float4*>(P_txt + static_cast<size_t>(t) * D);
  for (int i = threadIdx.x; i < n4; i += blockDim.x) {
    float4 a = e[i], c = p[i];
    xo[i] = make_float4(a.x + c.x, a.y + c.y, a.z + c.z, a.w + c.w);
  }
}

__global__ void __launch_bounds__(1024)
embed_depth_kernel(int trace_id, float* y, const float* E_top_depth, const float* P_depth, const int64_t* codes_top, int S, int pos,
                   int D) {
  TraceScope trace_scope(trace_id);
  pdl_launch_dependents();
  pdl_wait();
  const int b = blockIdx.x;
  const int64_t ct = codes_top[static_cast<size_t>(b) * S + pos];
  const float4* e = reinterpret_cast<const float4*>(E_top_depth + static_cast<size_t>(ct) * D);
  const float4* p = reinterpret_cast<const float4*>(P_depth);
  const int n4 = D / 4;
  for (int i = threadIdx.x; i < n4; i += blockDim.x) {
    const float4 a = e[i];
#pragma unroll
    for (int j = 0; j < 4; ++j) {
      const float4 c = p[j * n4 + i];
      reinterpret_cast<float4*>(y + (static_cast<size_t>(b) * 4 + j) * D)[i] =
          make_float4(a.x + c.x, a.y + c.y, a.z + c.z, a.w + c.w);
    }
  }
}

struct Embed3Args {
  float* x;
  const float* sos_table; const float* sos_override; const int64_t* cond;
  const float* E0; const float* E1; const float* E2; const float* P_top; const float* P_emb;
  const int64_t* codes_top;
  const int64_t* codes_mid;
  const int64_t* codes_bot;
  int D, S, pos, cond_kind;
};
__global__ void __launch_bounds__(1024) embed3_kernel(int trace_id, Embed3Args a) {
  TraceScope trace_scope(trace_id);
  pdl_launch_dependents();
  pdl_wait();
  const int b = blockIdx.x;
  float4* xo = reinterpret_cast<float4*>(a.x + static_cast<size_t>(b) * a.D);
  const int n4 = a.D / 4;
  if (a.pos == 0) {
    const float* src;
    if (a.sos_override != nullptr) src = a.sos_override + static_cast<size_t>(b) * a.D;
    else if (a.cond_kind == HQ_COND_CLS) src = a.sos_table + static_cast<size_t>(a.cond[b]) * a.D;
    else src = a.sos_table;
    const float4* s4 = reinterpret_cast<const float4*>(src);
    for (int i = threadIdx.x; i < n4; i += blockDim.x) xo[i] = s4[i];
    return;
  }
  const int p = a.pos - 1;
  __shared__ const float* rows[21];
  if (threadIdx.x < 21) {
    const size_t bp = static_cast<size_t>(b) * a.S + p;
    const int j = threadIdx.x;
    rows[j] = j == 0 ? a.E0 + static_cast<size_t>(a.codes_top[bp]) * a.D
            : j < 5 ? a.E1 + static_cast<size_t>(a.codes_mid[bp * 4 + (j - 1)]) * a.D
                    : a.E2 + static_cast<size_t>(a.codes_bot[bp * 16 + (j - 5)]) * a.D;
  }
  __syncthreads();
  const float4* pt = reinterpret_cast<const float4*>(a.P_top + static_cast<size_t>(p) * a.D);
  const float4* pe = reinterpret_cast<const float4*>(a.P_emb);
  for (int i = threadIdx.x; i < n4; i += blockDim.x) {
    const float4 t = reinterpret_cast<const float4*>(rows[0])[i], q = pt[i], e0 = pe[i];
    float4 acc;
    acc.x = (t.x + q.x) + e0.x; acc.y = (t.y + q.y) + e0.y; acc.z = (t.z + q.z) + e0.z; acc.w = (t.w + q.w) + e0.w;
#pragma unroll 4
    for (int j = 1; j < 21; ++j) {
      const float4 e = reinterpret_cast<const float4*>(rows[j])[i], pj = pe[j * n4 + i];
      acc.x += e.x + pj.x; acc.y += e.y + pj.y; acc.z += e.z + pj.z; acc.w += e.w + pj.w;
    }
    acc.x /= 21.0f; acc.y /= 21.0f; acc.z /= 21.0f; acc.w /= 21.0f;
    xo[i] = acc;
  }
}

__global__ void __launch_bounds__(1024)
embed_depth2_kernel(int trace_id, float* y, const float* E1d, const float* E0d, const float* P2, const int64_t* codes_top,
                    const int64_t* codes_mid, int S, int pos, int D) {
  TraceScope trace_scope(trace_id);
  pdl_launch_dependents();
  pdl_wait();
  const int b = blockIdx.x;
  const size_t bp = static_cast<size_t>(b) * S + pos;
  const float4* e0 = reinterpret_cast<const float4*>(E0d + static_cast<size_t>(codes_top[bp]) * D);
  const float4* em[4];
#pragma unroll
  for (int j = 0; j < 4; ++j) em[j] = reinterpret_cast<const float4*>(E1d + static_cast<size_t>(codes_mid[bp * 4 + j]) * D);
  const float4* p2 = reinterpret_cast<const float4*>(P2);
  const int n4 = D / 4;
  for (int i = threadIdx.x; i < n4; i += blockDim.x) {
    const float4 top = e0[i];
    float4 m[4];
#pragma unroll
    for (int j = 0; j < 4; ++j) m[j] = em[j][i];
#pragma unroll
    for (int t = 0; t < 16; ++t) {
      const float4 mm = m[((t >> 2) >> 1) * 2 + ((t & 3) >> 1)];
      const float4 pp = p2[t * n4 + i];
      reinterpret_cast<float4*>(y + (static_cast<size_t>(b) * 16 + t) * D)[i] =
          make_float4((mm.x + pp.x) + top.x, (mm.y + pp.y) + top.y, (mm.z + pp.z) + top.z, (mm.w + pp.w) + top.w);
    }
  }
}

template <typename AT>
__global__ void __launch_bounds__(256)
broadcast_prefix_kernel(int trace_id, AT* K, AT* V, float* yd, int Bmax, int Tc, int D) {
  TraceScope trace_scope(trace_id);
  pdl_launch_dependents();
  pdl_wait();
  const int t = blockIdx.x, l = blockIdx.y, b = blockIdx.z + 1;
  const size_t src = (static_cast<size_t>(l) * Bmax * Tc + t) * D;
  const size_t dst = ((static_cast<size_t>(l) * Bmax + b) * Tc + t) * D;
  constexpr int V8 = 16 / static_cast<int>(sizeof(AT));
  for (int i = threadIdx.x * V8; i < D; i += blockDim.x * V8) {
    *reinterpret_cast<uint4*>(K + dst + i) = *reinterpret_cast<const uint4*>(K + src + i);
    *reinterpret_cast<uint4*>(V + dst + i) = *reinterpret_cast<const uint4*>(V + src + i);
  }
  if (t == 0 && l == 0)
    for (int i = threadIdx.x * 4; i < D; i += blockDim.x * 4)
      *reinterpret_cast<float4*>(yd + static_cast<size_t>(b) * D + i) = *reinterpret_cast<const float4*>(yd + i);
}

__global__ void __launch_bounds__(1024)
embed_depth_seq_kernel(int trace_id, float* y, const float* E, const float* P_row, const int64_t* codes, int cstride, int D) {
  TraceScope trace_scope(trace_id);
  pdl_launch_dependents();
  pdl_wait();
  const int b = blockIdx.x;
  const int64_t c = codes[static_cast<size_t>(b) * cstride];
  const float4* e = reinterpret_cast<const float4*>(E + static_cast<size_t>(c) * D);
  const float4* p = reinterpret_cast<const float4*>(P_row);
  for (int i = threadIdx.x; i < D / 4; i += blockDim.x) {
    const float4 a = e[i], q = p[i];
    reinterpret_cast<float4*>(y + static_cast<size_t>(b) * D)[i] = make_float4(a.x + q.x, a.y + q.y, a.z + q.z, a.w + q.w);
  }
}

__global__ void __launch_bounds__(1024)
depth_pos_rows_kernel(int trace_id, float* y, const float* P_depth, int D) {
  TraceScope trace_scope(trace_id);
  pdl_launch_dependents();
  pdl_wait();
  const int b = blockIdx.x;
  const float4* p = reinterpret_cast<const float4*>(P_depth);
  const int n4 = D / 4;
  for (int i = threadIdx.x; i < n4; i += blockDim.x)
#pragma unroll
    for (int j = 0; j < 4; ++j) reinterpret_cast<float4*>(y + (static_cast<size_t>(b) * 5 + 1 + j) * D)[i] = p[j * n4 + i];
}

constexpr int LN_THREADS = 128;
constexpr int LN_MAXV = 3;
constexpr int LN_MAXFOLD = 6;

template <typename OutT>
__device__ __forceinline__ void ln_store4(OutT* o, int i, float y0, float y1, float y2, float y3) {
  if (sizeof(OutT) == 4) {
    *reinterpret_cast<float4*>(reinterpret_cast<float*>(o) + i) = make_float4(y0, y1, y2, y3);
  } else {
    uint2 u;
    __nv_bfloat162 h0 = __floats2bfloat162_rn(y0, y1), h1 = __floats2bfloat162_rn(y2, y3);
    u.x = *reinterpret_cast<uint32_t*>(&h0);
    u.y = *reinterpret_cast<uint32_t*>(&h1);
    *reinterpret_cast<uint2*>(reinterpret_cast<bf16*>(o) + i) = u;
  }
}

__device__ __forceinline__ float block_sum_128(float v, float* red ) {
  v = warp_sum(v);
  __syncthreads();
  if ((threadIdx.x & 31) == 0) red[threadIdx.x >> 5] = v;
  __syncthreads();
  return (red[0] + red[1]) + (red[2] + red[3]);
}

template <typename OutT, int MAXFOLD>
__global__ void __launch_bounds__(LN_THREADS)
layernorm_kernel(int trace_id, float* __restrict__ x, const float* __restrict__ gamma, const float* __restrict__ beta,
                 const float* __restrict__ add, OutT* __restrict__ out, int rows, int D, int in_mul, int in_off,
                 const float* __restrict__ fold, int n_fold, size_t fold_stride, const float* __restrict__ fold_bias,
                 int in_group, int out_mul) {
  TraceScope trace_scope(trace_id);
  pdl_launch_dependents();
  pdl_wait();
  __shared__ float red[4];
  const int r = blockIdx.x;
  const size_t in_row = static_cast<size_t>(r / in_group) * in_mul + in_off + (r % in_group);
  float* xr = x + in_row * D;
  OutT* o = out + static_cast<size_t>(r) * out_mul * D;
  const int tid = threadIdx.x;
  if (D <= LN_MAXV * LN_THREADS * 4) {
    float4 v[LN_MAXV], g[LN_MAXV], bt[LN_MAXV], ad[LN_MAXV], fb[LN_MAXV], f[MAXFOLD][LN_MAXV];
    const float4 z4 = make_float4(0.f, 0.f, 0.f, 0.f);
#pragma unroll
    for (int j = 0; j < LN_MAXV; ++j) {
      const int i = (j * LN_THREADS + tid) * 4;
      const int ic = i < D ? i : 0;
      v[j] = *reinterpret_cast<const float4*>(xr + ic);
      g[j] = *reinterpret_cast<const float4*>(gamma + ic);
      bt[j] = *reinterpret_cast<const float4*>(beta + ic);
      ad[j] = add != nullptr ? *reinterpret_cast<const float4*>(add + ic) : z4;
      fb[j] = z4;
#pragma unroll
      for (int sidx = 0; sidx < MAXFOLD; ++sidx) f[sidx][j] = z4;
      if (fold != nullptr) {
        const float* fr = fold + in_row * D + ic;
        fb[j] = fold_bias != nullptr ? *reinterpret_cast<const float4*>(fold_bias + ic) : z4;
#pragma unroll
        for (int sidx = 0; sidx < MAXFOLD; ++sidx)
          if (sidx < n_fold) f[sidx][j] = *reinterpret_cast<const float4*>(fr + sidx * fold_stride);
      }
    }
    float s = 0.f;
#pragma unroll
    for (int j = 0; j < LN_MAXV; ++j) {
      const int i = (j * LN_THREADS + tid) * 4;
      if (fold != nullptr) {
        float4 a = f[0][j];
#pragma unroll
        for (int sidx = 1; sidx < MAXFOLD; ++sidx) {
          a.x += f[sidx][j].x; a.y += f[sidx][j].y; a.z += f[sidx][j].z; a.w += f[sidx][j].w;
        }
        v[j].x += fb[j].x + a.x;
        v[j].y += fb[j].y + a.y;
        v[j].z += fb[j].z + a.z;
        v[j].w += fb[j].w + a.w;
        if (i < D) *reinterpret_cast<float4*>(xr + i) = v[j];
      }
      if (i < D) s += (v[j].x + v[j].y) + (v[j].z + v[j].w);
    }
    const float mean = block_sum_128(s, red) / static_cast<float>(D);
    float q = 0.f;
#pragma unroll
    for (int j = 0; j < LN_MAXV; ++j) {
      if ((j * LN_THREADS + tid) * 4 < D) {
        const float a = v[j].x - mean, b = v[j].y - mean, c = v[j].z - mean, d = v[j].w - mean;
        q += (a * a + b * b) + (c * c + d * d);
      }
    }
    const float rstd = 1.0f / sqrtf(block_sum_128(q, red) / static_cast<float>(D) + 1e-5f);
#pragma unroll
    for (int j = 0; j < LN_MAXV; ++j) {
      const int i = (j * LN_THREADS + tid) * 4;
      if (i < D) {
        ln_store4<OutT>(o, i, (v[j].x - mean) * rstd * g[j].x + bt[j].x + ad[j].x,
                        (v[j].y - mean) * rstd * g[j].y + bt[j].y + ad[j].y,
                        (v[j].z - mean) * rstd * g[j].z + bt[j].z + ad[j].z,
                        (v[j].w - mean) * rstd * g[j].w + bt[j].w + ad[j].w);
      }
    }
    return;
  }
  if (fold != nullptr) {
    for (int i = tid * 4; i < D; i += LN_THREADS * 4) {
      float4 v = *reinterpret_cast<const float4*>(xr + i);
      const float* fr = fold + in_row * D + i;
      float4 acc = *reinterpret_cast<const float4*>(fr);
      for (int sidx = 1; sidx < n_fold; ++sidx) {
        const float4 f = *reinterpret_cast<const float4*>(fr + sidx * fold_stride);
        acc.x += f.x; acc.y += f.y; acc.z += f.z; acc.w += f.w;
      }
      if (fold_bias != nullptr) {
        const float4 b = *reinterpret_cast<const float4*>(fold_bias + i);
        acc.x += b.x; acc.y += b.y; acc.z += b.z; acc.w += b.w;
      }
      v.x += acc.x; v.y += acc.y; v.z += acc.z; v.w += acc.w;
      *reinterpret_cast<float4*>(xr + i) = v;
    }
    __syncthreads();
  }
  float s = 0.f;
  for (int i = tid * 4; i < D; i += LN_THREADS * 4) {
    const float4 v = *reinterpret_cast<const float4*>(xr + i);
    s += (v.x + v.y) + (v.z + v.w);
  }
  const float mean = block_sum_128(s, red) / static_cast<float>(D);
  float q = 0.f;
  for (int i = tid * 4; i < D; i += LN_THREADS * 4) {
    const float4 v = *reinterpret_cast<const float4*>(xr + i);
    const float a = v.x - mean, b = v.y - mean, c = v.z - mean, d = v.w - mean;
    q += (a * a + b * b) + (c * c + d * d);
  }
  const float rstd = 1.0f / sqrtf(block_sum_128(q, red) / static_cast<float>(D) + 1e-5f);
  for (int i = tid * 4; i < D; i += LN_THREADS * 4) {
    const float4 v = *reinterpret_cast<const float4*>(xr + i);
    const float4 g = *reinterpret_cast<const float4*>(gamma + i);
    const float4 bt = *reinterpret_cast<const float4*>(beta + i);
    float y0 = (v.x - mean) * rstd * g.x + bt.x, y1 = (v.y - mean) * rstd * g.y + bt.y;
    float y2 = (v.z - mean) * rstd * g.z + bt.z, y3 = (v.w - mean) * rstd * g.w + bt.w;
    if (add != nullptr) {
      const float4 a4 = *reinterpret_cast<const float4*>(add + i);
      y0 += a4.x; y1 += a4.y; y2 += a4.z; y3 += a4.w;
    }
    ln_store4<OutT>(o, i, y0, y1, y2, y3);
  }
}

constexpr int ATT_MAX_KEYS = 128;
constexpr int ATT_WARPS = 8;

template <typename AT>
__global__ void __launch_bounds__(ATT_WARPS * 32)
attention_kernel(int trace_id, const AT* __restrict__ q, const AT* __restrict__ K, const AT* __restrict__ V, AT* __restrict__ out,
                 int M, int n_heads, int D, int Tq, int t_stride, int kbase, int causal) {
  TraceScope trace_scope(trace_id);
  pdl_launch_dependents();
  pdl_wait();
  __shared__ float sc[ATT_WARPS][ATT_MAX_KEYS];
  const int w = threadIdx.x >> 5, lane = threadIdx.x & 31;
  const int item = blockIdx.x * ATT_WARPS + w;
  if (item >= M * n_heads) return;
  const int m = item / n_heads, h = item % n_heads;
  const int b = m / Tq, i = m % Tq;
  const int n_keys = causal ? (kbase + i + 1) : kbase;
  const int g = lane >> 3, c = lane & 7;

  float qv[8];
  load8(q + static_cast<size_t>(m) * D + h * 64 + c * 8, qv);
  const AT* Kb = K + static_cast<size_t>(b) * t_stride * D + h * 64 + c * 8;
  const AT* Vb = V + static_cast<size_t>(b) * t_stride * D + h * 64 + c * 8;

#pragma unroll 4
  for (int tb = 0; tb < n_keys; tb += 4) {
    const int t = tb + g;
    float kv[8];
    if (t < n_keys) {
      load8_stream(Kb + static_cast<size_t>(t) * D, kv);
    } else {
#pragma unroll
      for (int e = 0; e < 8; ++e) kv[e] = 0.f;
    }
    float s = 0.f;
#pragma unroll
    for (int e = 0; e < 8; ++e) s = fmaf(qv[e], kv[e] * 0.125f, s);
    s += __shfl_xor_sync(0xffffffffu, s, 1);
    s += __shfl_xor_sync(0xffffffffu, s, 2);
    s += __shfl_xor_sync(0xffffffffu, s, 4);
    if (c == 0 && t < n_keys) sc[w][t] = s;
  }
  __syncwarp();
  float mx = -INFINITY;
  for (int t = lane; t < n_keys; t += 32) mx = fmaxf(mx, sc[w][t]);
  mx = warp_max(mx);
  float sum = 0.f;
  for (int t = lane; t < n_keys; t += 32) {
    const float e = expf(sc[w][t] - mx);
    sc[w][t] = e;
    sum += e;
  }
  sum = warp_sum(sum);
  __syncwarp();
  const float inv = 1.0f / sum;
  float acc[8];
#pragma unroll
  for (int e = 0; e < 8; ++e) acc[e] = 0.f;
#pragma unroll 4
  for (int t = g; t < n_keys; t += 4) {
    float vv[8];
    load8_stream(Vb + static_cast<size_t>(t) * D, vv);
    const float p = sc[w][t] * inv;
#pragma unroll
    for (int e = 0; e < 8; ++e) acc[e] = fmaf(p, vv[e], acc[e]);
  }
#pragma unroll
  for (int e = 0; e < 8; ++e) {
    acc[e] += __shfl_xor_sync(0xffffffffu, acc[e], 8);
    acc[e] += __shfl_xor_sync(0xffffffffu, acc[e], 16);
  }
  if (g == 0) store8(out + static_cast<size_t>(m) * D + h * 64 + c * 8, acc);
}

template <typename AT>
__global__ void __launch_bounds__(ATT_WARPS * 32)
attention_fewkeys_kernel(int trace_id, const AT* __restrict__ q, const AT* __restrict__ K, const AT* __restrict__ V,
                         AT* __restrict__ out, int M, int n_heads, int D, int Tq, int t_stride, int n_keys) {
  TraceScope trace_scope(trace_id);
  pdl_launch_dependents();
  pdl_wait();
// ... 234 lines not shown
    }
    __syncwarp();
    if (lane == 0) mbar_arrive(&empty_bar[s]);
  }
  if (threadIdx.x == 0) phase_mark(4);
  float mx = -INFINITY;
  for (int t = lane; t < n_keys; t += 32) mx = fmaxf(mx, row[t]);
  mx = warp_max(mx);
  float sum = 0.f;
  for (int t = lane; t < n_keys; t += 32) {
    const float e = expf(row[t] - mx);
    row[t] = e;
    sum += e;
  }
  const float inv = 1.0f / warp_sum(sum);
  __syncwarp();
  if (threadIdx.x == 0) phase_mark(5);
  float acc[8];
#pragma unroll
  for (int e = 0; e < 8; ++e) acc[e] = 0.f;
  for (; i < 2 * nck; ++i) {
    const int s = i % ATTD_STAGES;
    if (sleep_ns) mbar_wait_sleep(&full_bar[s], (i / ATTD_STAGES) & 1, sleep_ns);
    else mbar_wait(&full_bar[s], (i / ATTD_STAGES) & 1);
    const AT* st = reinterpret_cast<const AT*>(ring + s * stage_bytes) + w * 64 + c * 8;
    const int ck = i - nck;
    for (int kk = 0; kk < CH; kk += 4) {
      const int t = ck * CH + kk + g;
      if (t < n_keys) {
        float vv[8];
        load8(st + static_cast<size_t>(kk + g) * slice, vv);
        const float p = row[t] * inv;
#pragma unroll
        for (int e = 0; e < 8; ++e) acc[e] = fmaf(p, vv[e], acc[e]);
      }
    }
    __syncwarp();
    if (lane == 0) mbar_arrive(&empty_bar[s]);
  }
#pragma unroll
  for (int e = 0; e < 8; ++e) {
    acc[e] += __shfl_xor_sync(0xffffffffu, acc[e], 8);
    acc[e] += __shfl_xor_sync(0xffffffffu, acc[e], 16);
  }
  if (g == 0) store8(out + static_cast<size_t>(b) * D + h * 64 + c * 8, acc);
  if (threadIdx.x == 0) {
    phase_mark(6);
    phase_mark(7);
  }
#endif
}

constexpr int ATTM_CH = 8;
constexpr int ATTM_MAXSTAGES = 8;

__device__ __forceinline__ void ldmatrix_x2(uint32_t addr, uint32_t& r0, uint32_t& r1) {
#if defined(__CUDA_ARCH__)
  asm volatile("ldmatrix.sync.aligned.m8n8.x2.shared.b16 {%0,%1}, [%2];" : "=r"(r0), "=r"(r1) : "r"(addr));
#endif
}
__device__ __forceinline__ void ldmatrix_x2_trans(uint32_t addr, uint32_t& r0, uint32_t& r1) {
#if defined(__CUDA_ARCH__)
  asm volatile("ldmatrix.sync.aligned.m8n8.x2.trans.shared.b16 {%0,%1}, [%2];" : "=r"(r0), "=r"(r1) : "r"(addr));
#endif
}
__device__ __forceinline__ void mma_bf16_16816(float (&c)[4], uint32_t a0, uint32_t a1, uint32_t a2, uint32_t a3, uint32_t b0,
                                               uint32_t b1) {
#if defined(__CUDA_ARCH__)
  asm volatile("mma.sync.aligned.m16n8k16.row.col.f32.bf16.bf16.f32 {%0,%1,%2,%3}, {%4,%5,%6,%7}, {%8,%9}, {%0,%1,%2,%3};"
               : "+f"(c[0]), "+f"(c[1]), "+f"(c[2]), "+f"(c[3])
               : "r"(a0), "r"(a1), "r"(a2), "r"(a3), "r"(b0), "r"(b1));
#endif
}
__device__ __forceinline__ void mma_bf16_1688(float (&c)[4], uint32_t a0, uint32_t a1, uint32_t b0) {
#if defined(__CUDA_ARCH__)
  asm volatile("mma.sync.aligned.m16n8k8.row.col.f32.bf16.bf16.f32 {%0,%1,%2,%3}, {%4,%5}, {%6}, {%0,%1,%2,%3};"
               : "+f"(c[0]), "+f"(c[1]), "+f"(c[2]), "+f"(c[3])
               : "r"(a0), "r"(a1), "r"(b0));
#endif
}

__global__ void __launch_bounds__((ATTD_MAXHPC + 1) * 32)
attention_decode_mma_kernel(int trace_id, const __grid_constant__ CUtensorMap tmK, const __grid_constant__ CUtensorMap tmV,
                            int row_base, const bf16* __restrict__ q, bf16* __restrict__ out, int D, int t_stride, int n_keys,
                            int hpc, int groups, int n_items, int stages, unsigned int* __restrict__ sched) {
#if defined(__CUDA_ARCH__)
  TraceScope trace_scope(trace_id);
  const bool prefetch = stages > 0;
  if (stages < 0) stages = -stages;
  extern __shared__ uint8_t att_smem_raw[];
  uint8_t* ring = reinterpret_cast<uint8_t*>((reinterpret_cast<uintptr_t>(att_smem_raw) + 1023) & ~static_cast<uintptr_t>(1023));
  const int slice_bytes = hpc * 128;
  const int tile_bytes = ATTM_CH * slice_bytes;
  const int stage_bytes = 2 * tile_bytes;
  uint8_t* qbuf = ring + stages * stage_bytes;
  float* ostage = reinterpret_cast<float*>(qbuf + 2 * slice_bytes);
  uint64_t* full_bar = reinterpret_cast<uint64_t*>(ostage + hpc * 64);
  uint64_t* empty_bar = full_bar + ATTM_MAXSTAGES;
  uint64_t* qfull_bar = empty_bar + ATTM_MAXSTAGES;
  uint64_t* qempty_bar = qfull_bar + 2;
  int* qitem = reinterpret_cast<int*>(qempty_bar + 2);
  const int w = threadIdx.x >> 5, lane = threadIdx.x & 31;
  const int nck = (n_keys + ATTM_CH - 1) / ATTM_CH;
  if (threadIdx.x == 0) {
    phase_mark(0);
    tma_prefetch_desc(&tmK);
    tma_prefetch_desc(&tmV);
    for (int s = 0; s < stages; ++s) {
      mbar_init(&full_bar[s], 1);
      mbar_init(&empty_bar[s], hpc);
    }
    for (int s = 0; s < 2; ++s) {
      mbar_init(&qfull_bar[s], 1);
      mbar_init(&qempty_bar[s], hpc);
    }
    fence_barrier_init();
  }
  __syncthreads();
  if (threadIdx.x == 0) phase_mark(1);
  pdl_launch_dependents();

  if (w == hpc) {
    if (lane == 0) {
      bool waited = false;
      int item = blockIdx.x;
      uint32_t g = 0;
      for (int it = 0;; ++it) {
        const int ip = it & 1;
        const bool have = item < n_items;
        const int b = have ? item / groups : 0, grp = have ? item % groups : 0;
        const int row0 = row_base + b * t_stride;
        auto issue = [&](int ck, int s) {
          mbar_arrive_expect_tx(&full_bar[s], static_cast<uint32_t>(stage_bytes));
          uint8_t* dst = ring + s * stage_bytes;
          tma_load_3d(dst, &tmK, &full_bar[s], 0, grp * hpc, row0 + ck * ATTM_CH);
          tma_load_3d(dst + tile_bytes, &tmV, &full_bar[s], 0, grp * hpc, row0 + ck * ATTM_CH);
        };
        int i = 0;
        if (have && !waited && prefetch) {
          for (; i < nck - 1 && i < stages; ++i, ++g) issue(i, g % stages);
        }
        if (!waited) {
          pdl_wait();
          waited = true;
        }
        mbar_wait(&qempty_bar[ip], ((it >> 1) & 1) ^ 1);
        qitem[ip] = have ? item : -1;
        if (!have) {
          mbar_arrive(&qfull_bar[ip]);
          break;
        }
        if (it == 0) {
          mbar_arrive(&qfull_bar[ip]);
        } else {
          mbar_arrive_expect_tx(&qfull_bar[ip], slice_bytes);
          bulk_load_1d(qbuf + ip * slice_bytes, q + static_cast<size_t>(b) * D + grp * hpc * 64, slice_bytes, &qfull_bar[ip]);
        }
        const int next = static_cast<int>(atomicAdd(sched, 1u)) + static_cast<int>(gridDim.x);
        for (; i < nck; ++i, ++g) {
          const int s = g % stages;
          mbar_wait(&empty_bar[s], ((g / stages) & 1) ^ 1);
          issue(i, s);
        }
        item = next;
      }
      if (atomicAdd(sched + 1, 1u) == gridDim.x - 1) {
        sched[0] = 0;
        sched[1] = 0;
        __threadfence();
      }
    }
    return;
  }
  if (w > hpc) return;

  pdl_wait();
  const int gq = lane >> 2, tq = lane & 3;
  const int lr = lane & 7, lm = (lane >> 3) & 1;
  const uint32_t ring_u32 = smem_u32(ring);
  uint32_t frag_off[4];
  {
    const uint32_t line = static_cast<uint32_t>(lr * hpc + w);
#pragma unroll
    for (int j = 0; j < 4; ++j) frag_off[j] = line * 128u + (((2u * j + lm) ^ (line & 7u)) << 4);
  }
  float* orow = ostage + w * 64;
  uint32_t g = 0;
  for (int it = 0;; ++it) {
    const int ip = it & 1;
    mbar_wait(&qfull_bar[ip], (it >> 1) & 1);
    const int item = qitem[ip];
    if (item < 0) break;
    uint32_t qb[4][2];
    {
      const uint32_t* q32 =
          it == 0 ? reinterpret_cast<const uint32_t*>(q + static_cast<size_t>(item / groups) * D + ((item % groups) * hpc + w) * 64)
                  : reinterpret_cast<const uint32_t*>(qbuf + ip * slice_bytes + w * 128);
#pragma unroll
      for (int ks = 0; ks < 4; ++ks) {
        qb[ks][0] = gq == 0 ? q32[ks * 8 + tq] : 0u;
        qb[ks][1] = gq == 0 ? q32[ks * 8 + 4 + tq] : 0u;
      }
    }
    if (it == 0 && threadIdx.x == 0) phase_mark(2);
    __syncwarp();
    if (lane == 0) mbar_arrive(&qempty_bar[ip]);

    float m_run = -INFINITY, l_run = 0.f;
    float o[4][4];
#pragma unroll
    for (int mt = 0; mt < 4; ++mt)
#pragma unroll
      for (int e = 0; e < 4; ++e) o[mt][e] = 0.f;

    for (int c = 0; c < nck; ++c, ++g) {
      const int s = g % stages;
      const int left = n_keys - c * ATTM_CH;
      mbar_wait(&full_bar[s], (g / stages) & 1);
      if (g == 0 && threadIdx.x == 0) phase_mark(3);
// ... 273 lines not shown
    {
      float cum = above;
      while (keep_ties < n_ties && cum < top_p) { ++keep_ties; cum += vstar; }
      if (keep_ties == 0) keep_ties = 1;
    }
    int tie_before = 0;
    if (keep_ties < n_ties) {
      const int lane = tid & 31, w = tid >> 5, nw = nthr >> 5;
      int incl = ties;
#pragma unroll
      for (int o = 1; o < 32; o <<= 1) {
        const int n = __shfl_up_sync(0xffffffffu, incl, o);
        if (lane >= o) incl += n;
      }
      __syncthreads();
      if (lane == 31) iscratch[w] = incl;
      __syncthreads();
      int woff = 0;
      for (int k2 = 0; k2 < w && k2 < nw; ++k2) woff += iscratch[k2];
      tie_before = woff + incl - ties;
      __syncthreads();
    }
    float ksum = 0.f;
#pragma unroll
    for (int i = 0; i < SMP_IPT; ++i) {
      const uint32_t u = __float_as_uint(wgt[i]);
      bool keep = u > cstar;
      if (u == cstar && wgt[i] > 0.f) { keep = tie_before < keep_ties; ++tie_before; }
      if (!keep) wgt[i] = 0.f;
      ksum += wgt[i];
    }
    ksum = block_reduce(ksum, OpSumF(), 0.f, fscratch);
    const float inv = 1.0f / ksum;
#pragma unroll
    for (int i = 0; i < SMP_IPT; ++i) wgt[i] *= inv;
  }
  if (a.probs_out != nullptr) {
#pragma unroll
    for (int i = 0; i < SMP_IPT; ++i)
      if (i < ipt && base + i < V) a.probs_out[static_cast<size_t>(r) * V + base + i] = wgt[i];
  }

  float local = 0.f;
#pragma unroll
  for (int i = 0; i < SMP_IPT; ++i) local += wgt[i];
  float excl, total;
  {
    const int lane = tid & 31, w = tid >> 5, nw = nthr >> 5;
    float incl = local;
#pragma unroll
    for (int o = 1; o < 32; o <<= 1) {
      const float n = __shfl_up_sync(0xffffffffu, incl, o);
      if (lane >= o) incl += n;
    }
    __syncthreads();
    if (lane == 31) wsum[w] = incl;
    __syncthreads();
    float woff = 0.f, tot = 0.f;
    for (int k2 = 0; k2 < nw; ++k2) {
      if (k2 < w) woff += wsum[k2];
      tot += wsum[k2];
    }
    float prev = __shfl_up_sync(0xffffffffu, incl, 1);
    if (lane == 0) prev = 0.f;
    excl = woff + prev;
    total = tot;
  }
  const uint64_t grow = row_offset + static_cast<uint64_t>(b);
  uint32_t rnd[4];
  philox4x32_10(static_cast<uint32_t>(seed), static_cast<uint32_t>(seed >> 32), static_cast<uint32_t>(grow),
                static_cast<uint32_t>(grow >> 32), static_cast<uint32_t>(a.pos), static_cast<uint32_t>(slot), rnd);
  const float target = u01_from_bits(rnd[0]) * total;
  int cand = -1;
  float run = excl;
#pragma unroll
  for (int i = 0; i < SMP_IPT; ++i) {
    if (wgt[i] > 0.f && run <= target) cand = base + i;
    run += wgt[i];
  }
  cand = block_reduce(cand, OpMaxI(), -1, iscratch);
  if (tid == 0) *dst = cand;
}

constexpr int SMPF_WARPS = 8;
__global__ void __launch_bounds__(SMPF_WARPS * 32) sample_finalize_kernel(int trace_id, SampleArgs a, const float2* __restrict__ part,
                                                                          int n_chunks) {
  TraceScope trace_scope(trace_id);
  pdl_launch_dependents();
  pdl_wait();
  const int lane = threadIdx.x & 31;
  const int r = blockIdx.x * SMPF_WARPS + (threadIdx.x >> 5);
  if (r >= a.R) return;
  const int b = r / a.rows_per_b, jj = r % a.rows_per_b;
  const int slot = a.slot0 + jj;
  const float2* p = part + static_cast<size_t>(r) * n_chunks;
  const int per = (n_chunks + 31) / 32;
  const int c0 = lane * per, c1 = min(n_chunks, c0 + per);
  float mx = -INFINITY;
  for (int c = c0; c < c1; ++c) mx = fmaxf(mx, p[c].x);
#pragma unroll
  for (int o = 16; o > 0; o >>= 1) mx = fmaxf(mx, __shfl_xor_sync(0xffffffffu, mx, o));
  float local = 0.f;
  for (int c = c0; c < c1; ++c) local += expf(p[c].x - mx);
  float incl = local;
#pragma unroll
  for (int o = 1; o < 32; o <<= 1) {
    const float n = __shfl_up_sync(0xffffffffu, incl, o);
    if (lane >= o) incl += n;
  }
  const float total = __shfl_sync(0xffffffffu, incl, 31);
  const uint64_t seed = a.sp->seed, grow = a.sp->row_offset + static_cast<uint64_t>(b);
  uint32_t rnd[4];
  philox4x32_10(static_cast<uint32_t>(seed), static_cast<uint32_t>(seed >> 32), static_cast<uint32_t>(grow),
                static_cast<uint32_t>(grow >> 32), static_cast<uint32_t>(a.pos), static_cast<uint32_t>(slot) | 0x100u, rnd);
  const float target = u01_from_bits(rnd[0]) * total;
  int cand = -1;
  float run = incl - local;
  for (int c = c0; c < c1; ++c) {
    const float w = expf(p[c].x - mx);
    if (w > 0.f && run <= target) cand = c;
    run += w;
  }
#pragma unroll
  for (int o = 16; o > 0; o >>= 1) cand = max(cand, __shfl_xor_sync(0xffffffffu, cand, o));
  if (lane == 0) {
    int64_t* dst = a.dst_codes + (static_cast<size_t>(b) * a.S + a.pos) * a.dst_w +
                   (a.rows_per_b == 1 ? (a.bot_slot < 0 ? 0 : a.bot_slot) : jj);
    *dst = static_cast<int64_t>(__float_as_int(p[cand < 0 ? 0 : cand].y));
  }
}

}
```

### hqtransformer_b200/engine.py

```python
from __future__ import annotations

import ctypes as C
from dataclasses import dataclass
from typing import Dict, Optional, Sequence, Union

import torch

from . import _lib
from ._lib import HQConfig, HQRunArgs, HQSamplingParams, check

_TORCH2HQ = {torch.float32: _lib.HQ_F32, torch.bfloat16: _lib.HQ_BF16, torch.float16: _lib.HQ_F16}


@dataclass
class SamplingParams:
    top_k_top: Optional[int] = None
    top_p_top: Optional[float] = None
    top_k_bot: Optional[int] = None
    top_p_bot: Optional[float] = None
    temperature_top: float = 1.0
    temperature_bot: float = 1.0
    seed: int = 0
    row_offset: int = 0
    top_k_mid: Optional[int] = None
# ... 157 lines not shown
        import numpy as np
        args = HQRunArgs(batch=batch, seq_len=seq_len, pos_begin=pos_begin, pos_end=pos_end, cond=_ptr(cond), sos=None,
                         given_top=None, given_bot=None, codes_top=_ptr(codes_top), codes_bot=_ptr(codes_bot),
                         logits=None, sampling=sampling.to_c())
        out = (C.c_uint64 * (2 * max_entries))()
        tags = C.create_string_buffer(48 * max_entries)
        ph = (C.c_uint64 * (max_ctas * 16))()
        n = C.c_int()
        st = torch.cuda.current_stream(self.device).cuda_stream
        check(self._lib.hq_debug_gemm_phases(self._ctx, C.byref(args), C.c_void_p(st), launch_id, ph, max_ctas, out, tags,
                                             max_entries, C.byref(n)), self._ctx, "hq_debug_gemm_phases")
        raw = tags.raw
        tl = [(raw[48 * i:48 * i + 48].split(b"\0")[0].decode(), int(out[2 * i]), int(out[2 * i + 1])) for i in range(n.value)]
        return tl, np.frombuffer(ph, dtype=np.uint64).reshape(max_ctas, 16).astype(np.int64)

    def bench_attention(self, batch: int, n_keys: int, iters: int = 50) -> float:
        us = C.c_float()
        st = torch.cuda.current_stream(self.device).cuda_stream
        check(self._lib.hq_bench_attention(self._ctx, batch, n_keys, iters, C.byref(us), C.c_void_p(st)), self._ctx,
              "hq_bench_attention")
        return us.value

    def attention_phases(self, batch: int, n_keys: int, warm: int = 3, max_ctas: int = 4096):
        import numpy as np
        buf = (C.c_uint64 * (max_ctas * 8))()
        n = C.c_int()
        st = torch.cuda.current_stream(self.device).cuda_stream
        check(self._lib.hq_debug_attention_phases(self._ctx, batch, n_keys, warm, buf, max_ctas, C.byref(n), C.c_void_p(st)),
              self._ctx, "hq_debug_attention_phases")
        return np.frombuffer(buf, dtype=np.uint64).reshape(max_ctas, 8)[:n.value].astype(np.int64)

    def chain_phases(self, *, batch: int, seq_len: int, pos_begin: int, pos_end: int, sampling: SamplingParams,
                     cond: Optional[torch.Tensor], codes_top: torch.Tensor, codes_bot: torch.Tensor, launch_idx: int,
                     op_idx: int, max_ctas: int = 256):
        import numpy as np
        args = HQRunArgs(batch=batch, seq_len=seq_len, pos_begin=pos_begin, pos_end=pos_end, cond=_ptr(cond), sos=None,
                         given_top=None, given_bot=None, codes_top=_ptr(codes_top), codes_bot=_ptr(codes_bot),
                         logits=None, sampling=sampling.to_c())
        buf = (C.c_uint64 * (max_ctas * 8))()
        n = C.c_int()
        st = torch.cuda.current_stream(self.device).cuda_stream
        check(self._lib.hq_debug_chain_phases(self._ctx, C.byref(args), C.c_void_p(st), launch_idx, op_idx, buf, max_ctas,
                                              C.byref(n)), self._ctx, "hq_debug_chain_phases")
        return np.frombuffer(buf, dtype=np.uint64).reshape(max_ctas, 8)[:n.value].astype(np.int64)

    def bench_gemm(self, kind: int, M: int, iters: int = 20) -> float:
        us = C.c_float()
        st = torch.cuda.current_stream(self.device).cuda_stream
        check(self._lib.hq_bench_gemm(self._ctx, kind, M, iters, C.byref(us), C.c_void_p(st)), self._ctx,
              "hq_bench_gemm")
        return us.value


def debug_gemm(A: torch.Tensor, W: torch.Tensor, tile: int = 0) -> torch.Tensor:
    lib = _lib.load()
    assert A.is_cuda and W.is_cuda and A.dtype == W.dtype and A.is_contiguous() and W.is_contiguous()
    M, K = A.shape
    N = W.shape[0]
    out = torch.empty(M, N, dtype=torch.float32, device=A.device)
    prec = _lib.HQ_PREC_BF16 if A.dtype == torch.bfloat16 else _lib.HQ_PREC_FP32
    with torch.cuda.device(A.device):
        st = torch.cuda.current_stream(A.device).cuda_stream
        check(lib.hq_debug_gemm(prec, A.data_ptr(), W.data_ptr(), out.data_ptr(), M, N, K, tile, C.c_void_p(st)), None,
              "hq_debug_gemm")
    return out


def debug_attention(q: torch.Tensor, K: torch.Tensor, V: torch.Tensor, n_keys: int, variant: int = 0) -> torch.Tensor:
    lib = _lib.load()
    assert q.is_cuda and q.dtype == K.dtype == V.dtype and q.dtype in (torch.bfloat16, torch.float32)
    assert q.is_contiguous() and K.is_contiguous() and V.is_contiguous() and K.shape == V.shape
    B, D = q.shape
    T = K.shape[1]
    assert K.shape == (B, T, D) and D % 64 == 0 and 1 <= n_keys <= T
    out = torch.empty_like(q)
    prec = _lib.HQ_PREC_BF16 if q.dtype == torch.bfloat16 else _lib.HQ_PREC_FP32
    with torch.cuda.device(q.device):
        st = torch.cuda.current_stream(q.device).cuda_stream
        check(lib.hq_debug_attention(prec, q.data_ptr(), K.data_ptr(), V.data_ptr(), out.data_ptr(), B, D // 64, T, n_keys,
                                     variant, C.c_void_p(st)), None, "hq_debug_attention")
    return out


def debug_philox(seed: int, counter: Sequence[int]):
    lib = _lib.load()
    c = (C.c_uint32 * 4)(*counter)
    o = (C.c_uint32 * 4)()
    check(lib.hq_debug_philox(seed, c, o), None, "hq_debug_philox")
    return [int(v) for v in o]


def debug_sample(logits: torch.Tensor, temperature: float = 1.0, top_k: Optional[int] = None,
                 top_p: Optional[float] = None, seed: int = 0, row_offset: int = 0, position: int = 0, slot: int = 0,
                 return_probs: bool = False):
    lib = _lib.load()
    assert logits.is_cuda and logits.dtype == torch.float32 and logits.is_contiguous() and logits.dim() == 2
    R, V = logits.shape
    codes = torch.empty(R, dtype=torch.int64, device=logits.device)
    probs = torch.empty(R, V, dtype=torch.float32, device=logits.device) if return_probs else None
    with torch.cuda.device(logits.device):
        st = torch.cuda.current_stream(logits.device).cuda_stream
        check(lib.hq_debug_sample(logits.data_ptr(), R, V, float(temperature), int(top_k) if top_k else 0,
                                  float(top_p) if top_p is not None else 0.0, seed, row_offset, position, slot,
                                  codes.data_ptr(), _ptr(probs), C.c_void_p(st)), None, "hq_debug_sample")
    return (codes, probs) if return_probs else codes


def bench_gemm_shape(M: int, N: int, K: int, tile: int = 0, iters: int = 20, flush: int = 2, copies: int = 1):
    lib = _lib.load()
    mean, mn = C.c_float(), C.c_float()
    st = torch.cuda.current_stream().cuda_stream
    check(lib.hq_bench_gemm_shape(M, N, K, tile, iters, flush, copies, C.byref(mean), C.byref(mn), C.c_void_p(st)), None,
          "hq_bench_gemm_shape")
    return mean.value, mn.value
```

### include/hqgraft.h

```cpp
#ifndef HQGRAFT_H_
#define HQGRAFT_H_

#include <stddef.h>
#include <stdint.h>

#ifdef __cplusplus
extern "C" {
#endif

#define HQ_ABI_VERSION 8

enum hq_status {
  HQ_OK = 0,
  HQ_ERR_INVALID = 1,
  HQ_ERR_CUDA = 2,
  HQ_ERR_UNSUPPORTED = 3,
  HQ_ERR_STATE = 4
};

enum hq_cond_kind { HQ_COND_CLS = 0, HQ_COND_TXT = 1, HQ_COND_UNCOND = 2 };

enum hq_precision { HQ_PREC_BF16 = 0, HQ_PREC_FP32 = 1 };

enum hq_dtype { HQ_F32 = 0, HQ_BF16 = 1, HQ_F16 = 2 };
// ... 23 lines not shown
  int32_t use_chain;
  int32_t model_type;
  int32_t embedding_kind;
  int32_t position_kind;
  int32_t code_levels;
  int32_t vocab_mid;
  int32_t fuse_head_sampler;
} hq_config;

typedef struct hq_sampling_params {
  int32_t top_k_top;
  int32_t top_k_bot;
  float top_p_top;
  float top_p_bot;
  float temperature_top;
  float temperature_bot;
  uint64_t seed;
  uint64_t row_offset;
  int32_t top_k_mid;
  float top_p_mid;
  float temperature_mid;
  int32_t reserved;
} hq_sampling_params;

typedef struct hq_run_args {
  int32_t batch;
  int32_t seq_len;
  int32_t pos_begin;
  int32_t pos_end;
  const int64_t* cond;
  const float* sos;
  const int64_t* given_top;
  const int64_t* given_bot;
  int64_t* codes_top;
  int64_t* codes_bot;
  float* logits;
  hq_sampling_params sampling;
  int64_t* codes_mid;
  const int64_t* given_mid;
  int32_t shared_prefix;
  int32_t reserved;
} hq_run_args;

typedef struct hq_ctx hq_ctx;

int hq_abi_version(void);

const char* hq_last_error(const hq_ctx* ctx);

int hq_create(const hq_config* cfg, int device, int max_batch, hq_ctx** out);

int hq_destroy(hq_ctx* ctx);

int hq_reserve_batch(hq_ctx* ctx, int max_batch);
int hq_max_batch(const hq_ctx* ctx);

int hq_load_param(hq_ctx* ctx, const char* name, const void* data, int dtype,
                  const int64_t* shape, int ndim, int is_device);

int hq_params_complete(hq_ctx* ctx);

int hq_run(hq_ctx* ctx, const hq_run_args* args, void* stream);

int hq_run_host(hq_ctx* ctx, const hq_run_args* args);

int64_t hq_last_launch_count(const hq_ctx* ctx);

int64_t hq_chain_launch_count(const hq_ctx* ctx);

size_t hq_device_bytes(const hq_ctx* ctx);


int hq_debug_gemm(int prec, const void* A, const void* W, float* C, int M, int N, int K, int tile, void* stream);

int hq_debug_philox(uint64_t seed, const uint32_t counter[4], uint32_t out[4]);

int hq_debug_sample(const float* logits, int R, int V, float temperature, int top_k, float top_p,
                    uint64_t seed, uint64_t row_offset, int position, int slot,
                    int64_t* out_codes, float* out_probs , void* stream);

int hq_debug_attention(int prec, const void* q, const void* K, const void* V, void* out, int B, int n_heads,
                       int t_stride, int n_keys, int variant, void* stream);

int hq_bench_attention(hq_ctx* ctx, int B, int n_keys, int iters, float* usec, void* stream);

int hq_debug_attention_phases(hq_ctx* ctx, int B, int n_keys, int warm, unsigned long long* out_ns, int max_ctas,
                              int* n_ctas, void* stream);

int hq_debug_chain_phases(hq_ctx* ctx, const hq_run_args* args, void* stream, int launch_idx, int op_idx,
                          unsigned long long* out_ns, int max_ctas, int* n_ctas);

int hq_bench_gemm(hq_ctx* ctx, int kind, int M, int iters, float* usec, void* stream);

int hq_trace_run(hq_ctx* ctx, const hq_run_args* args, void* stream, unsigned long long* out_ns, char* tags,
                 int max_entries, int* n_entries);

int hq_debug_gemm_phases(hq_ctx* ctx, const hq_run_args* args, void* stream, int launch_id, unsigned long long* phases,
                         int max_ctas, unsigned long long* out_ns, char* tags, int max_entries, int* n_entries);

int hq_bench_gemm_shape(int M, int N, int K, int tile, int iters, int flush, int copies, float* usec_mean,
                        float* usec_min, void* stream);

typedef struct hq_s1_config {
  int32_t embed_dim;
  int32_t n_embed;
  int32_t z_channels;
  int32_t resolution;
  int32_t ch;
  int32_t ch_mult[8];
  int32_t n_levels;
  int32_t num_res_blocks;
  int32_t attn_resolution;
  int32_t out_ch;
} hq_s1_config;

typedef struct hq_s1_ctx hq_s1_ctx;

int hq_s1_create(const hq_s1_config* cfg, int device, int max_batch, hq_s1_ctx** out);
int hq_s1_destroy(hq_s1_ctx* ctx);
const char* hq_s1_last_error(const hq_s1_ctx* ctx);
size_t hq_s1_device_bytes(const hq_s1_ctx* ctx);

int hq_s1_load_param(hq_s1_ctx* ctx, const char* name, const void* data, int dtype, const int64_t* shape, int ndim,
                     int is_device);
int hq_s1_params_complete(hq_s1_ctx* ctx);

int hq_s1_decode_codes(hq_s1_ctx* ctx, const int64_t* code_t, const int64_t* code_b, float* out, int B, void* stream);

double hq_s1_last_conv_flops(const hq_s1_ctx* ctx);

#ifdef __cplusplus
}
#endif
#endif
```

Measured before the change: 3526.

## Fuse embeddings and final layernorms into next block's first layernorm; trim attention tail loads

Embedding kernels, the final layernorm, and the top-code sample finalize/depth-embed now also compute the following block's first layernorm, so run_block can skip that separate layernorm launch. The aim is to remove several small kernel launches and a full-row reread per decode step. Attention decode also gets per-tail-size TMA maps, so the last key chunk loads only the rows it needs instead of a full chunk. In exchange there are more kernel variants, extra tensor maps, and tighter coupling: several fused paths are off when chain recording or shared-prefix mode is active.

```diff
diff --git a/hqtransformer_b200/_lib.py b/hqtransformer_b200/_lib.py
--- a/hqtransformer_b200/_lib.py
+++ b/hqtransformer_b200/_lib.py
@@ -66,6 +66,8 @@
                                   C.c_int, C.c_int, C.c_void_p, C.c_void_p, C.c_void_p]),
     "hq_debug_attention": (C.c_int, [C.c_int, C.c_void_p, C.c_void_p, C.c_void_p, C.c_void_p, C.c_int, C.c_int, C.c_int,
                                      C.c_int, C.c_int, C.c_void_p]),
+    "hq_debug_layernorm": (C.c_int, [C.c_int, C.c_void_p, C.c_void_p, C.c_void_p, C.c_void_p, C.c_void_p, C.c_int, C.c_void_p,
+                                     C.c_void_p, C.c_void_p, C.c_void_p, C.c_void_p, C.c_int, C.c_int, C.c_void_p]),
     "hq_debug_attention_phases": (C.c_int, [C.c_void_p, C.c_int, C.c_int, C.c_int, C.POINTER(C.c_uint64), C.c_int,
                                             C.POINTER(C.c_int), C.c_void_p]),
     "hq_debug_chain_phases": (C.c_int, [C.c_void_p, C.POINTER(HQRunArgs), C.c_void_p, C.c_int, C.c_int, C.POINTER(C.c_uint64),
diff --git a/hqtransformer_b200/csrc/engine.cu b/hqtransformer_b200/csrc/engine.cu
--- a/hqtransformer_b200/csrc/engine.cu
+++ b/hqtransformer_b200/csrc/engine.cu
@@ -169,7 +169,7 @@
   float2* samp_part = nullptr;
   float* splitk_ws = nullptr;
   unsigned int* att_sched = nullptr;
-  CUtensorMap kmap, vmap;
+  CUtensorMap kmap[ATTM_CH], vmap[ATTM_CH];
   bool kv_maps = false;
   int num_sms = 0;
   int ws_rows = 0;
@@ -284,18 +284,20 @@
   return HQ_OK;
 }
 
-static int make_kv_map(hq_ctx* ctx, CUtensorMap* m, const void* base, int n_heads, uint64_t rows, int hpc) {
-  cuuint64_t dims[3] = {64, static_cast<cuuint64_t>(n_heads), rows};
-  cuuint64_t strides[2] = {128, static_cast<cuuint64_t>(n_heads) * 128};
-  cuuint32_t box[3] = {64, static_cast<cuuint32_t>(hpc), 8};
-  cuuint32_t estr[3] = {1, 1, 1};
-  CUresult r = ctx->encode(m, CU_TENSOR_MAP_DATA_TYPE_BFLOAT16, 3, const_cast<void*>(base), dims, strides, box, estr,
-                           CU_TENSOR_MAP_INTERLEAVE_NONE, CU_TENSOR_MAP_SWIZZLE_128B, CU_TENSOR_MAP_L2_PROMOTION_L2_256B,
-                           CU_TENSOR_MAP_FLOAT_OOB_FILL_NONE);
-  if (r != CUDA_SUCCESS) {
-    set_err(ctx, "cuTensorMapEncodeTiled (KV cache) failed (%d) heads=%d rows=%llu hpc=%d", static_cast<int>(r), n_heads,
-            static_cast<unsigned long long>(rows), hpc);
-    return HQ_ERR_CUDA;
+static int make_kv_maps(hq_ctx* ctx, CUtensorMap (&m)[ATTM_CH], const void* base, int n_heads, uint64_t rows, int hpc) {
+  for (int r = 0; r < ATTM_CH; ++r) {
+    cuuint64_t dims[3] = {64, static_cast<cuuint64_t>(n_heads), rows};
+    cuuint64_t strides[2] = {128, static_cast<cuuint64_t>(n_heads) * 128};
+    cuuint32_t box[3] = {64, static_cast<cuuint32_t>(hpc), static_cast<cuuint32_t>(r == 0 ? ATTM_CH : r)};
+    cuuint32_t estr[3] = {1, 1, 1};
+    CUresult e = ctx->encode(&m[r], CU_TENSOR_MAP_DATA_TYPE_BFLOAT16, 3, const_cast<void*>(base), dims, strides, box, estr,
+                             CU_TENSOR_MAP_INTERLEAVE_NONE, CU_TENSOR_MAP_SWIZZLE_128B, CU_TENSOR_MAP_L2_PROMOTION_L2_256B,
+                             CU_TENSOR_MAP_FLOAT_OOB_FILL_NONE);
+    if (e != CUDA_SUCCESS) {
+      set_err(ctx, "cuTensorMapEncodeTiled (KV cache) failed (%d) heads=%d rows=%llu hpc=%d box_rows=%d", static_cast<int>(e),
+              n_heads, static_cast<unsigned long long>(rows), hpc, r);
+      return HQ_ERR_CUDA;
+    }
   }
   return HQ_OK;
 }
@@ -523,8 +525,8 @@
     const int groups = attn_groups(ctx, ctx->nh);
     if (groups > 0) {
       const uint64_t rows = static_cast<uint64_t>(ctx->L) * B * ctx->Tc;
-      if ((rc = make_kv_map(ctx, &ctx->kmap, ctx->kc, ctx->nh, rows, ctx->nh / groups))) return rc;
-      if ((rc = make_kv_map(ctx, &ctx->vmap, ctx->vc, ctx->nh, rows, ctx->nh / groups))) return rc;
+      if ((rc = make_kv_maps(ctx, ctx->kmap, ctx->kc, ctx->nh, rows, ctx->nh / groups))) return rc;
+      if ((rc = make_kv_maps(ctx, ctx->vmap, ctx->vc, ctx->nh, rows, ctx->nh / groups))) return rc;
       ctx->kv_maps = true;
     }
   }
@@ -1196,9 +1198,10 @@
 void launch_attn_mma<bf16>(hq_ctx* ctx, cudaStream_t st, const bf16* q, const bf16* K, bf16* out, int t_stride, int n_keys,
                            int hpc, int groups, int n_items, int stages, int grid, size_t smem) {
   const int row_base = static_cast<int>((K - static_cast<const bf16*>(ctx->kc)) / ctx->D);
-  launch_k(ctx, st, "attention_decode", attention_decode_mma_kernel, dim3(grid), dim3((hpc + 1) * 32), smem, ctx->kmap, ctx->vmap,
-           row_base, q, out, ctx->D, t_stride, n_keys, hpc, groups, n_items, attn_prefetch_ok(ctx) ? stages : -stages,
-           ctx->att_sched);
+  const int tail = n_keys % ATTM_CH;
+  launch_k(ctx, st, "attention_decode", attention_decode_mma_kernel, dim3(grid), dim3((hpc + 1) * 32), smem, ctx->kmap[0],
+           ctx->vmap[0], ctx->kmap[tail], ctx->vmap[tail], row_base, q, out, ctx->D, t_stride, n_keys, hpc, groups, n_items,
+           attn_prefetch_ok(ctx) ? stages : -stages, ctx->att_sched);
 }
 
 template <typename AT>
@@ -1330,13 +1333,13 @@
 
 template <typename AT>
 static void run_block(hq_ctx* ctx, cudaStream_t st, const BlockW& w, float* x, int M, int mode, AT* kdst, AT* vdst,
-                      int rpb, int t_stride, int t0, int n_keys_base, int causal, Fold* fold) {
+                      int rpb, int t_stride, int t0, int n_keys_base, int causal, Fold* fold, bool h_ready = false) {
   const int D = ctx->D;
   AT* h = static_cast<AT*>(ctx->h.ptr);
   AT* att = static_cast<AT*>(ctx->att.ptr);
   AT* mlp = static_cast<AT*>(ctx->mlp.ptr);
   AT* q = static_cast<AT*>(ctx->q);
-  layernorm_act<AT>(ctx, st, x, w.ln1g, w.ln1b, h, M, fold);
+  if (!h_ready) layernorm_act<AT>(ctx, st, x, w.ln1g, w.ln1b, h, M, fold);
   EpiParams<AT> ep;
   memset(&ep, 0, sizeof(ep));
   ep.q = q; ep.kdst = kdst; ep.vdst = vdst; ep.D = D; ep.rpb = rpb; ep.t_stride = t_stride; ep.t0 = t0;
@@ -1411,9 +1414,10 @@
   const int eb = (D / 4 + 31) / 32 * 32 > 1024 ? 1024 : (D / 4 + 31) / 32 * 32;
   Fold fold_x, fold_y;
   ctx->full_dependency_next = true;
+  const BlockW& w0 = ctx->blocks[0];
   if (prefill) {
-    launch_k(ctx, st, "embed_txt", embed_txt_kernel, dim3(M), dim3(eb), 0, ctx->x, f.sos_override ? ctx->sos_override : nullptr,
-             ctx->cond, ctx->E_txt, ctx->P_txt, T0, D);
+    launch_k(ctx, st, "embed_txt_ln", embed_txt_ln_kernel<AT>, dim3(M), dim3(LN_THREADS), 0, ctx->x,
+             f.sos_override ? ctx->sos_override : nullptr, ctx->cond, ctx->E_txt, ctx->P_txt, T0, D, w0.ln1g, w0.ln1b, h);
   } else {
     EmbedArgs ea;
     ea.x = ctx->x; ea.sos_table = ctx->sos_table; ea.sos_override = f.sos_override ? ctx->sos_override : nullptr;
@@ -1421,17 +1425,27 @@
     ea.codes_top = ctx->codes_top; ea.codes_bot = ctx->codes_bot; ea.D = D; ea.S = S; ea.pos = pos;
     ea.cond_kind = ctx->cfg.cond_kind;
     ea.emb_kind = ctx->cfg.embedding_kind; ea.P_top_h = ctx->P_top_h; ea.P_top_w = ctx->P_top_w; ea.Hpos = ctx->Hpos;
-    launch_k(ctx, st, "embed", embed_kernel, dim3(B), dim3(eb), 0, ea);
+    launch_k(ctx, st, "embed_ln", embed_ln_kernel<AT>, dim3(B), dim3(LN_THREADS), 0, ea, w0.ln1g, w0.ln1b, h);
   }
 
   const int tok = (pos == 0) ? 0 : T0 + pos - 1;
   const bool chain = sizeof(AT) == 2 && !prefill && chain_enabled(ctx, B);
   if (chain) chain_begin(ctx, tok, pos, S);
   for (int l = 0; l < ctx->L; ++l) {
-    if (prefill) run_block<AT>(ctx, st, ctx->blocks[l], ctx->x, M, 0, kc + l * lstride, vc + l * lstride, T0, Tc, 0, 0, 1, &fold_x);
-    else run_block<AT>(ctx, st, ctx->blocks[l], ctx->x, M, 0, kc + l * lstride, vc + l * lstride, 1, Tc, tok, tok + 1, 0, &fold_x);
-  }
-  if (ctx->recording) {
+    if (prefill)
+      run_block<AT>(ctx, st, ctx->blocks[l], ctx->x, M, 0, kc + l * lstride, vc + l * lstride, T0, Tc, 0, 0, 1, &fold_x, l == 0);
+    else
+      run_block<AT>(ctx, st, ctx->blocks[l], ctx->x, M, 0, kc + l * lstride, vc + l * lstride, 1, Tc, tok, tok + 1, 0, &fold_x,
+                    l == 0);
+  }
+  const bool depth_h_ready = !ctx->recording && !shared && (ctx->cfg.model_type == HQ_MODEL_PARALLEL ||
+                                                              ctx->cfg.model_type == HQ_MODEL_TOP2BOT);
+  if (depth_h_ready) {
+    const BlockW& d0 = ctx->depths[0];
+    launch_k(ctx, st, "layernorm_f_ln", fold_x.n > 3 ? layernorm2_kernel<AT, LN_MAXFOLD> : layernorm2_kernel<AT, 3>, dim3(B),
+             dim3(LN_THREADS), 0, ctx->x, ctx->lnf_g, ctx->lnf_b, ctx->sos_depth, ctx->yd, D, prefill ? T0 : 1,
+             prefill ? T0 - 1 : 0, fold_x.partial, fold_x.n, fold_x.stride, fold_x.bias, d0.ln1g, d0.ln1b, h);
+  } else if (ctx->recording) {
     ChainOp* op = chain_push(ctx, CH_OP_LN, "layernorm_f");
     op->flags = CH_F_OUT_F32;
     op->x = ctx->x; op->gamma = ctx->lnf_g; op->beta = ctx->lnf_b; op->add = ctx->sos_depth; op->out = ctx->yd;
@@ -1463,7 +1477,8 @@
                  static_cast<const float*>(ctx->P_depth + static_cast<size_t>(c - 1) * D), codes, c == 1 ? S : 4 * S, D);
       }
       for (int l = 0; l < ctx->Ld; ++l)
-        run_block<AT>(ctx, st, ctx->depths[l], ctx->yd, B, 0, kd + l * dstride, vd + l * dstride, 1, 5, c, c + 1, 0, &fold_y);
+        run_block<AT>(ctx, st, ctx->depths[l], ctx->yd, B, 0, kd + l * dstride, vd + l * dstride, 1, 5, c, c + 1, 0, &fold_y,
+                      c == 0 && l == 0 && depth_h_ready);
       layernorm_act<AT>(ctx, st, ctx->yd, c == 0 ? ctx->lnt_g : ctx->lnb_g, c == 0 ? ctx->lnt_b : ctx->lnb_b, h, B, &fold_y);
       sa.V = c == 0 ? ctx->Vt : ctx->Vb; sa.slot0 = c; sa.bot_slot = c - 1;
       sa.dst_codes = c == 0 ? ctx->codes_top : ctx->codes_bot; sa.dst_w = c == 0 ? 1 : 4;
@@ -1489,24 +1504,35 @@
   }
 
   for (int l = 0; l < ctx->Ld; ++l)
-    run_block<AT>(ctx, st, ctx->depths[l], ctx->yd, B, 1, kd + l * dstride, vd + l * dstride, 1, 5, 0, 1, 0, &fold_y);
+    run_block<AT>(ctx, st, ctx->depths[l], ctx->yd, B, 1, kd + l * dstride, vd + l * dstride, 1, 5, 0, 1, 0, &fold_y,
+                  l == 0 && depth_h_ready);
   layernorm_act<AT>(ctx, st, ctx->yd, ctx->lnt_g, ctx->lnt_b, h, B, &fold_y);
+  bool depth1_h_ready = false;
   {
     const bool fused = head_gemm<AT>(ctx, st, ctx->head_top, B, ctx->Vt, sa, f);
     if (chain) chain_end(ctx, st);
-    draw(ctx, st, sa, fused);
+    depth1_h_ready = fused && !chain;
+    if (depth1_h_ready) {
+      const BlockW& d0 = ctx->depths[0];
+      launch_k(ctx, st, "sample_finalize_depth", sample_finalize_depth_kernel<AT>, dim3(B), dim3(LN_THREADS), 0, sa,
+               static_cast<const float2*>(ctx->samp_part), sa.V / 32, ctx->yd, ctx->E_top_depth, ctx->P_depth, D, d0.ln1g,
+               d0.ln1b, h);
+    } else {
+      draw(ctx, st, sa, fused);
+    }
   }
 
   if (chain) {
     chain_begin(ctx, tok, pos, S);
     ChainOp* op = chain_push(ctx, CH_OP_EMBED_DEPTH, "embed_depth");
     op->y = ctx->yd; op->E = ctx->E_top_depth; op->P = ctx->P_depth; op->codes_top = ctx->codes_top; op->B = B; op->D = D;
-  } else {
+  } else if (!depth1_h_ready) {
     launch_k(ctx, st, "embed_depth", embed_depth_kernel, dim3(B), dim3(eb), 0, ctx->yd, ctx->E_top_depth, ctx->P_depth,
              ctx->codes_top, S, pos, D);
   }
   for (int l = 0; l < ctx->Ld; ++l)
-    run_block<AT>(ctx, st, ctx->depths[l], ctx->yd, 4 * B, 2, kd + l * dstride, vd + l * dstride, 4, 5, 1, 5, 0, &fold_y);
+    run_block<AT>(ctx, st, ctx->depths[l], ctx->yd, 4 * B, 2, kd + l * dstride, vd + l * dstride, 4, 5, 1, 5, 0, &fold_y,
+                  l == 0 && depth1_h_ready);
   layernorm_act<AT>(ctx, st, ctx->yd, ctx->lnb_g, ctx->lnb_b, h, 4 * B, &fold_y);
   sa.V = ctx->Vb; sa.R = 4 * B; sa.rows_per_b = 4; sa.slot0 = 1; sa.forced = f.forced_bot;
   sa.temp_sel = 1; sa.filt_sel = 1; sa.dst_codes = ctx->codes_bot; sa.dst_w = 4;
@@ -1795,8 +1821,8 @@
     tmp.kc = const_cast<void*>(K);
     tmp.vc = const_cast<void*>(V);
     if ((rc = get_encode_fn(&tmp, &tmp.encode)) == HQ_OK && groups > 0 &&
-        (rc = make_kv_map(&tmp, &tmp.kmap, K, n_heads, static_cast<uint64_t>(B) * t_stride, n_heads / groups)) == HQ_OK &&
-        (rc = make_kv_map(&tmp, &tmp.vmap, V, n_heads, static_cast<uint64_t>(B) * t_stride, n_heads / groups)) == HQ_OK)
+        (rc = make_kv_maps(&tmp, tmp.kmap, K, n_heads, static_cast<uint64_t>(B) * t_stride, n_heads / groups)) == HQ_OK &&
+        (rc = make_kv_maps(&tmp, tmp.vmap, V, n_heads, static_cast<uint64_t>(B) * t_stride, n_heads / groups)) == HQ_OK)
       tmp.kv_maps = true;
     if (rc) {
       cudaFree(tmp.att_sched);
@@ -1911,6 +1937,35 @@
   launch_sample(&tmp, static_cast<cudaStream_t>(stream), sa);
   if (tmp.launch_err != cudaSuccess) {
     set_err(nullptr, "hq_debug_sample launch failed: %s", cudaGetErrorString(tmp.launch_err));
+    return HQ_ERR_CUDA;
+  }
+  return HQ_OK;
+}
+
+extern "C" int hq_debug_layernorm(int fused, float* x, const float* gamma, const float* beta, const float* add,
+                                  const float* fold, int n_fold, const float* fold_bias, const float* gamma2,
+                                  const float* beta2, float* y, void* h, int rows, int D, void* stream) {
+  if (!x || !gamma || !beta || !gamma2 || !beta2 || !y || !h || rows < 1 || D < 4 || D % 4 != 0 || n_fold < 0 ||
+      n_fold > LN_MAXFOLD || (n_fold > 0) != (fold != nullptr)) {
+    set_err(nullptr, "hq_debug_layernorm: bad argument");
+    return HQ_ERR_INVALID;
+  }
+  hq_ctx tmp;
+  cudaStream_t st = static_cast<cudaStream_t>(stream);
+  const size_t fstride = static_cast<size_t>(rows) * D;
+  bf16* hb = static_cast<bf16*>(h);
+  if (fused) {
+    launch_k(&tmp, st, "layernorm_f_ln", n_fold > 3 ? layernorm2_kernel<bf16, LN_MAXFOLD> : layernorm2_kernel<bf16, 3>,
+             dim3(rows), dim3(LN_THREADS), 0, x, gamma, beta, add, y, D, 1, 0, fold, n_fold, fstride, fold_bias, gamma2, beta2, hb);
+  } else {
+    launch_k(&tmp, st, "layernorm_f", n_fold > 3 ? layernorm_kernel<float, LN_MAXFOLD> : layernorm_kernel<float, 3>, dim3(rows),
+             dim3(LN_THREADS), 0, x, gamma, beta, add, y, rows, D, 1, 0, fold, n_fold, fstride, fold_bias, 1, 1);
+    launch_k(&tmp, st, "layernorm", layernorm_kernel<bf16, 3>, dim3(rows), dim3(LN_THREADS), 0, y, gamma2, beta2,
+             static_cast<const float*>(nullptr), hb, rows, D, 1, 0, static_cast<const float*>(nullptr), 0, size_t(0),
+             static_cast<const float*>(nullptr), 1, 1);
+  }
+  if (tmp.launch_err != cudaSuccess) {
+    set_err(nullptr, "hq_debug_layernorm launch failed: %s", cudaGetErrorString(tmp.launch_err));
     return HQ_ERR_CUDA;
   }
   return HQ_OK;
diff --git a/hqtransformer_b200/csrc/kernels.cuh b/hqtransformer_b200/csrc/kernels.cuh
--- a/hqtransformer_b200/csrc/kernels.cuh
+++ b/hqtransformer_b200/csrc/kernels.cuh
@@ -20,7 +20,118 @@
   int Hpos;
 };
 
-__global__ void __launch_bounds__(1024) embed_kernel(int trace_id, EmbedArgs a) {
+struct EmbedSrc {
+  static constexpr bool kComputed = true;
+  const float4* s4;
+  const float4* et; const float4* pt; const float4* pw; const float4* pe; const float4* eb[4]; const float* ebq[4];
+  int n4, emb_kind;
+  __device__ __forceinline__ EmbedSrc(const EmbedArgs& a, int b) {
+    n4 = a.D / 4;
+    emb_kind = a.emb_kind;
+    s4 = nullptr;
+    if (a.pos == 0) {
+      const float* src;
+      if (a.sos_override != nullptr) src = a.sos_override + static_cast<size_t>(b) * a.D;
+      else if (a.cond_kind == HQ_COND_CLS) src = a.sos_table + static_cast<size_t>(a.cond[b]) * a.D;
+      else src = a.sos_table;
+      s4 = reinterpret_cast<const float4*>(src);
+      return;
+    }
+    const int p = a.pos - 1;
+    const int64_t ct = a.codes_top[static_cast<size_t>(b) * a.S + p];
+    const int64_t* cbp = a.codes_bot + (static_cast<size_t>(b) * a.S + p) * 4;
+    et = reinterpret_cast<const float4*>(a.E_top + static_cast<size_t>(ct) * a.D);
+    const bool pos2d = a.P_top_h != nullptr;
+    pt = reinterpret_cast<const float4*>(pos2d ? a.P_top_h + static_cast<size_t>(p / a.Hpos) * a.D
+                                               : a.P_top + static_cast<size_t>(p) * a.D);
+    pw = pos2d ? reinterpret_cast<const float4*>(a.P_top_w + static_cast<size_t>(p % a.Hpos) * a.D) : nullptr;
+    pe = reinterpret_cast<const float4*>(a.P_emb);
+#pragma unroll
+    for (int j = 0; j < 4; ++j) {
+      eb[j] = reinterpret_cast<const float4*>(a.E_bot + static_cast<size_t>(cbp[j]) * a.D);
+      ebq[j] = a.E_bot + static_cast<size_t>(cbp[j]) * (a.D / 4);
+    }
+  }
+  __device__ __forceinline__ float4 operator()(const float*, int ic) const {
+    const int i = ic >> 2;
+    if (s4 != nullptr) return s4[i];
+    const float4 t = et[i];
+    float4 q = pt[i];
+    if (pw != nullptr) { const float4 w = pw[i]; q.x += w.x; q.y += w.y; q.z += w.z; q.w += w.w; }
+    if (emb_kind == 1) {
+      return make_float4((t.x + q.x) + ebq[0][i], (t.y + q.y) + ebq[1][i], (t.z + q.z) + ebq[2][i], (t.w + q.w) + ebq[3][i]);
+    }
+    const float4 e0 = pe[i];
+    float4 acc;
+    acc.x = (t.x + q.x) + e0.x; acc.y = (t.y + q.y) + e0.y; acc.z = (t.z + q.z) + e0.z; acc.w = (t.w + q.w) + e0.w;
+#pragma unroll
+    for (int j = 0; j < 4; ++j) {
+      const float4 e = eb[j][i], pj = pe[(j + 1) * n4 + i];
+      acc.x += e.x + pj.x; acc.y += e.y + pj.y; acc.z += e.z + pj.z; acc.w += e.w + pj.w;
+    }
+    acc.x /= 5.0f; acc.y /= 5.0f; acc.z /= 5.0f; acc.w /= 5.0f;
+    return acc;
+  }
+};
+
+struct EmbedTxtSrc {
+  static constexpr bool kComputed = true;
+  const float4* s4; const float4* e; const float4* p;
+  __device__ __forceinline__ EmbedTxtSrc(const float* sos_override, const int64_t* ids, const float* E_txt, const float* P_txt,
+                                         int T, int D, int row) {
+    s4 = sos_override != nullptr ? reinterpret_cast<const float4*>(sos_override + static_cast<size_t>(row) * D) : nullptr;
+    e = s4 != nullptr ? nullptr : reinterpret_cast<const float4*>(E_txt + static_cast<size_t>(ids[row]) * D);
+    p = reinterpret_cast<const float4*>(P_txt + static_cast<size_t>(row % T) * D);
+  }
+  __device__ __forceinline__ float4 operator()(const float*, int ic) const {
+    const int i = ic >> 2;
+    if (s4 != nullptr) return s4[i];
+    const float4 a = e[i], c = p[i];
+    return make_float4(a.x + c.x, a.y + c.y, a.z + c.z, a.w + c.w);
+  }
+};
+
+struct EmbedDepthSrc {
+  static constexpr bool kComputed = true;
+  const float4* e; const float4* p;
+  __device__ __forceinline__ float4 operator()(const float*, int ic) const {
+    const float4 a = e[ic >> 2], c = p[ic >> 2];
+    return make_float4(a.x + c.x, a.y + c.y, a.z + c.z, a.w + c.w);
+  }
+};
+
+__global__ void __launch_bounds__(1024)
+embed_depth_kernel(int trace_id, float* y, const float* E_top_depth, const float* P_depth, const int64_t* codes_top, int S, int pos,
+                   int D) {
+  TraceScope trace_scope(trace_id);
+  pdl_launch_dependents();
+  pdl_wait();
+  const int b = blockIdx.x;
+  const int64_t ct = codes_top[static_cast<size_t>(b) * S + pos];
+  const float4* e = reinterpret_cast<const float4*>(E_top_depth + static_cast<size_t>(ct) * D);
+  const float4* p = reinterpret_cast<const float4*>(P_depth);
+  const int n4 = D / 4;
+  for (int i = threadIdx.x; i < n4; i += blockDim.x) {
+    const float4 a = e[i];
+#pragma unroll
+    for (int j = 0; j < 4; ++j) {
+      const float4 c = p[j * n4 + i];
+      reinterpret_cast<float4*>(y + (static_cast<size_t>(b) * 4 + j) * D)[i] =
+          make_float4(a.x + c.x, a.y + c.y, a.z + c.z, a.w + c.w);
+    }
+  }
+}
+
+struct Embed3Args {
+  float* x;
+  const float* sos_table; const float* sos_override; const int64_t* cond;
+  const float* E0; const float* E1; const float* E2; const float* P_top; const float* P_emb;
+  const int64_t* codes_top;
+  const int64_t* codes_mid;
+  const int64_t* codes_bot;
+  int D, S, pos, cond_kind;
+};
+__global__ void __launch_bounds__(1024) embed3_kernel(int trace_id, Embed3Args a) {
   TraceScope trace_scope(trace_id);
   pdl_launch_dependents();
   pdl_wait();
@@ -37,116 +148,6 @@
     return;
   }
   const int p = a.pos - 1;
-  const int64_t ct = a.codes_top[static_cast<size_t>(b) * a.S + p];
-  const int64_t* cbp = a.codes_bot + (static_cast<size_t>(b) * a.S + p) * 4;
-  const float4* et = reinterpret_cast<const float4*>(a.E_top + static_cast<size_t>(ct) * a.D);
-  const bool pos2d = a.P_top_h != nullptr;
-  const float4* pt = reinterpret_cast<const float4*>(pos2d ? a.P_top_h + static_cast<size_t>(p / a.Hpos) * a.D
-                                                           : a.P_top + static_cast<size_t>(p) * a.D);
-  const float4* pw = pos2d ? reinterpret_cast<const float4*>(a.P_top_w + static_cast<size_t>(p % a.Hpos) * a.D) : nullptr;
-  if (a.emb_kind == 1) {
-    const int Dq = a.D / 4;
-    const float* ebq[4];
-#pragma unroll
-    for (int j = 0; j < 4; ++j) ebq[j] = a.E_bot + static_cast<size_t>(cbp[j]) * Dq;
-    for (int i = threadIdx.x; i < n4; i += blockDim.x) {
-      const float4 t = et[i];
-      float4 q = pt[i];
-      if (pos2d) { const float4 w = pw[i]; q.x += w.x; q.y += w.y; q.z += w.z; q.w += w.w; }
-      xo[i] = make_float4((t.x + q.x) + ebq[0][i], (t.y + q.y) + ebq[1][i], (t.z + q.z) + ebq[2][i], (t.w + q.w) + ebq[3][i]);
-    }
-    return;
-  }
-  const float4* eb[4];
-#pragma unroll
-  for (int j = 0; j < 4; ++j) eb[j] = reinterpret_cast<const float4*>(a.E_bot + static_cast<size_t>(cbp[j]) * a.D);
-  const float4* pe = reinterpret_cast<const float4*>(a.P_emb);
-  for (int i = threadIdx.x; i < n4; i += blockDim.x) {
-    float4 t = et[i], q = pt[i], e0 = pe[i];
-    if (pos2d) { const float4 w = pw[i]; q.x += w.x; q.y += w.y; q.z += w.z; q.w += w.w; }
-    float4 acc;
-    acc.x = (t.x + q.x) + e0.x; acc.y = (t.y + q.y) + e0.y; acc.z = (t.z + q.z) + e0.z; acc.w = (t.w + q.w) + e0.w;
-#pragma unroll
-    for (int j = 0; j < 4; ++j) {
-      float4 e = eb[j][i], pj = pe[(j + 1) * n4 + i];
-      acc.x += e.x + pj.x; acc.y += e.y + pj.y; acc.z += e.z + pj.z; acc.w += e.w + pj.w;
-    }
-    acc.x /= 5.0f; acc.y /= 5.0f; acc.z /= 5.0f; acc.w /= 5.0f;
-    xo[i] = acc;
-  }
-}
-
-__global__ void __launch_bounds__(1024)
-embed_txt_kernel(int trace_id, float* x, const float* sos_override, const int64_t* ids, const float* E_txt, const float* P_txt,
-                 int T, int D) {
-  TraceScope trace_scope(trace_id);
-  pdl_launch_dependents();
-  pdl_wait();
-  const int row = blockIdx.x;
-  const int t = row % T;
-  float4* xo = reinterpret_cast<float4*>(x + static_cast<size_t>(row) * D);
-  const int n4 = D / 4;
-  if (sos_override != nullptr) {
-    const float4* s4 = reinterpret_cast<const float4*>(sos_override + static_cast<size_t>(row) * D);
-    for (int i = threadIdx.x; i < n4; i += blockDim.x) xo[i] = s4[i];
-    return;
-  }
-  const float4* e = reinterpret_cast<const float4*>(E_txt + static_cast<size_t>(ids[row]) * D);
-  const float4* p = reinterpret_cast<const float4*>(P_txt + static_cast<size_t>(t) * D);
-  for (int i = threadIdx.x; i < n4; i += blockDim.x) {
-    float4 a = e[i], c = p[i];
-    xo[i] = make_float4(a.x + c.x, a.y + c.y, a.z + c.z, a.w + c.w);
-  }
-}
-
-__global__ void __launch_bounds__(1024)
-embed_depth_kernel(int trace_id, float* y, const float* E_top_depth, const float* P_depth, const int64_t* codes_top, int S, int pos,
-                   int D) {
-  TraceScope trace_scope(trace_id);
-  pdl_launch_dependents();
-  pdl_wait();
-  const int b = blockIdx.x;
-  const int64_t ct = codes_top[static_cast<size_t>(b) * S + pos];
-  const float4* e = reinterpret_cast<const float4*>(E_top_depth + static_cast<size_t>(ct) * D);
-  const float4* p = reinterpret_cast<const float4*>(P_depth);
-  const int n4 = D / 4;
-  for (int i = threadIdx.x; i < n4; i += blockDim.x) {
-    const float4 a = e[i];
-#pragma unroll
-    for (int j = 0; j < 4; ++j) {
-      const float4 c = p[j * n4 + i];
-      reinterpret_cast<float4*>(y + (static_cast<size_t>(b) * 4 + j) * D)[i] =
-          make_float4(a.x + c.x, a.y + c.y, a.z + c.z, a.w + c.w);
-    }
-  }
-}
-
-struct Embed3Args {
-  float* x;
-  const float* sos_table; const float* sos_override; const int64_t* cond;
-  const float* E0; const float* E1; const float* E2; const float* P_top; const float* P_emb;
-  const int64_t* codes_top;
-  const int64_t* codes_mid;
-  const int64_t* codes_bot;
-  int D, S, pos, cond_kind;
-};
-__global__ void __launch_bounds__(1024) embed3_kernel(int trace_id, Embed3Args a) {
-  TraceScope trace_scope(trace_id);
-  pdl_launch_dependents();
-  pdl_wait();
-  const int b = blockIdx.x;
-  float4* xo = reinterpret_cast<float4*>(a.x + static_cast<size_t>(b) * a.D);
-  const int n4 = a.D / 4;
-  if (a.pos == 0) {
-    const float* src;
-    if (a.sos_override != nullptr) src = a.sos_override + static_cast<size_t>(b) * a.D;
-    else if (a.cond_kind == HQ_COND_CLS) src = a.sos_table + static_cast<size_t>(a.cond[b]) * a.D;
-    else src = a.sos_table;
-    const float4* s4 = reinterpret_cast<const float4*>(src);
-    for (int i = threadIdx.x; i < n4; i += blockDim.x) xo[i] = s4[i];
-    return;
-  }
-  const int p = a.pos - 1;
   __shared__ const float* rows[21];
   if (threadIdx.x < 21) {
     const size_t bp = static_cast<size_t>(b) * a.S + p;
@@ -273,20 +274,16 @@
   return (red[0] + red[1]) + (red[2] + red[3]);
 }
 
-template <typename OutT, int MAXFOLD>
-__global__ void __launch_bounds__(LN_THREADS)
-layernorm_kernel(int trace_id, float* __restrict__ x, const float* __restrict__ gamma, const float* __restrict__ beta,
-                 const float* __restrict__ add, OutT* __restrict__ out, int rows, int D, int in_mul, int in_off,
-                 const float* __restrict__ fold, int n_fold, size_t fold_stride, const float* __restrict__ fold_bias,
-                 int in_group, int out_mul) {
-  TraceScope trace_scope(trace_id);
-  pdl_launch_dependents();
-  pdl_wait();
-  __shared__ float red[4];
-  const int r = blockIdx.x;
-  const size_t in_row = static_cast<size_t>(r / in_group) * in_mul + in_off + (r % in_group);
-  float* xr = x + in_row * D;
-  OutT* o = out + static_cast<size_t>(r) * out_mul * D;
+struct LnStoredRow {
+  static constexpr bool kComputed = false;
+  __device__ __forceinline__ float4 operator()(const float* xr, int ic) const { return *reinterpret_cast<const float4*>(xr + ic); }
+};
+template <typename OutT, int MAXFOLD, typename Src = LnStoredRow>
+__device__ __forceinline__ void layernorm_row(float* __restrict__ xr, const float* __restrict__ gamma,
+                                              const float* __restrict__ beta, const float* __restrict__ add,
+                                              OutT* __restrict__ o, int D, const float* __restrict__ fold, size_t in_row,
+                                              int n_fold, size_t fold_stride, const float* __restrict__ fold_bias, float* red ,
+                                              const Src& src = Src()) {
   const int tid = threadIdx.x;
   if (D <= LN_MAXV * LN_THREADS * 4) {
     float4 v[LN_MAXV], g[LN_MAXV], bt[LN_MAXV], ad[LN_MAXV], fb[LN_MAXV], f[MAXFOLD][LN_MAXV];
@@ -295,7 +292,7 @@
     for (int j = 0; j < LN_MAXV; ++j) {
       const int i = (j * LN_THREADS + tid) * 4;
       const int ic = i < D ? i : 0;
-      v[j] = *reinterpret_cast<const float4*>(xr + ic);
+      v[j] = src(xr, ic);
       g[j] = *reinterpret_cast<const float4*>(gamma + ic);
       bt[j] = *reinterpret_cast<const float4*>(beta + ic);
       ad[j] = add != nullptr ? *reinterpret_cast<const float4*>(add + ic) : z4;
@@ -325,6 +322,8 @@
         v[j].z += fb[j].z + a.z;
         v[j].w += fb[j].w + a.w;
         if (i < D) *reinterpret_cast<float4*>(xr + i) = v[j];
+      } else if (Src::kComputed) {
+        if (i < D) *reinterpret_cast<float4*>(xr + i) = v[j];
       }
       if (i < D) s += (v[j].x + v[j].y) + (v[j].z + v[j].w);
     }
@@ -349,6 +348,10 @@
       }
     }
     return;
+  }
+  if (Src::kComputed) {
+    for (int i = tid * 4; i < D; i += LN_THREADS * 4) *reinterpret_cast<float4*>(xr + i) = src(xr, i);
+    __syncthreads();
   }
   if (fold != nullptr) {
     for (int i = tid * 4; i < D; i += LN_THREADS * 4) {
@@ -393,6 +396,66 @@
     }
     ln_store4<OutT>(o, i, y0, y1, y2, y3);
   }
+}
+
+template <typename OutT, int MAXFOLD>
+__global__ void __launch_bounds__(LN_THREADS)
+layernorm_kernel(int trace_id, float* __restrict__ x, const float* __restrict__ gamma, const float* __restrict__ beta,
+                 const float* __restrict__ add, OutT* __restrict__ out, int rows, int D, int in_mul, int in_off,
+                 const float* __restrict__ fold, int n_fold, size_t fold_stride, const float* __restrict__ fold_bias,
+                 int in_group, int out_mul) {
+  TraceScope trace_scope(trace_id);
+  pdl_launch_dependents();
+  pdl_wait();
+  __shared__ float red[4];
+  const int r = blockIdx.x;
+  const size_t in_row = static_cast<size_t>(r / in_group) * in_mul + in_off + (r % in_group);
+  layernorm_row<OutT, MAXFOLD>(x + in_row * D, gamma, beta, add, out + static_cast<size_t>(r) * out_mul * D, D, fold, in_row,
+                               n_fold, fold_stride, fold_bias, red);
+}
+
+template <typename OutT>
+__global__ void __launch_bounds__(LN_THREADS)
+embed_ln_kernel(int trace_id, EmbedArgs a, const float* __restrict__ gamma, const float* __restrict__ beta, OutT* __restrict__ h) {
+  TraceScope trace_scope(trace_id);
+  pdl_launch_dependents();
+  pdl_wait();
+  __shared__ float red[4];
+  const int b = blockIdx.x;
+  layernorm_row<OutT, 3>(a.x + static_cast<size_t>(b) * a.D, gamma, beta, nullptr, h + static_cast<size_t>(b) * a.D, a.D,
+                         nullptr, 0, 0, 0, nullptr, red, EmbedSrc(a, b));
+}
+
+template <typename OutT>
+__global__ void __launch_bounds__(LN_THREADS)
+embed_txt_ln_kernel(int trace_id, float* x, const float* sos_override, const int64_t* ids, const float* E_txt,
+                    const float* P_txt, int T, int D, const float* __restrict__ gamma, const float* __restrict__ beta,
+                    OutT* __restrict__ h) {
+  TraceScope trace_scope(trace_id);
+  pdl_launch_dependents();
+  pdl_wait();
+  __shared__ float red[4];
+  const int row = blockIdx.x;
+  layernorm_row<OutT, 3>(x + static_cast<size_t>(row) * D, gamma, beta, nullptr, h + static_cast<size_t>(row) * D, D, nullptr,
+                         0, 0, 0, nullptr, red, EmbedTxtSrc(sos_override, ids, E_txt, P_txt, T, D, row));
+}
+
+template <typename OutT, int MAXFOLD>
+__global__ void __maxnreg__(MAXFOLD > 3 ? 152 : 112)
+layernorm2_kernel(int trace_id, float* __restrict__ x, const float* __restrict__ gamma, const float* __restrict__ beta,
+                  const float* __restrict__ add, float* __restrict__ y, int D, int in_mul, int in_off,
+                  const float* __restrict__ fold, int n_fold, size_t fold_stride, const float* __restrict__ fold_bias,
+                  const float* __restrict__ gamma2, const float* __restrict__ beta2, OutT* __restrict__ h) {
+  TraceScope trace_scope(trace_id);
+  pdl_launch_dependents();
+  pdl_wait();
+  __shared__ float red[4];
+  const int r = blockIdx.x;
+  const size_t in_row = static_cast<size_t>(r) * in_mul + in_off;
+  float* yr = y + static_cast<size_t>(r) * D;
+  layernorm_row<float, MAXFOLD>(x + in_row * D, gamma, beta, add, yr, D, fold, in_row, n_fold, fold_stride, fold_bias, red);
+  __syncthreads();
+  layernorm_row<OutT, 3>(yr, gamma2, beta2, nullptr, h + static_cast<size_t>(r) * D, D, nullptr, 0, 0, 0, nullptr, red);
 }
 
 constexpr int ATT_MAX_KEYS = 128;
@@ -793,7 +856,7 @@
 
 __global__ void __launch_bounds__((ATTD_MAXHPC + 1) * 32)
 attention_decode_mma_kernel(int trace_id, const __grid_constant__ CUtensorMap tmK, const __grid_constant__ CUtensorMap tmV,
-                            int row_base, const bf16* __restrict__ q, bf16* __restrict__ out, int D, int t_stride, int n_keys,
+                            const __grid_constant__ CUtensorMap tmKt, const __grid_constant__ CUtensorMap tmVt, int row_base, const bf16* __restrict__ q, bf16* __restrict__ out, int D, int t_stride, int n_keys,
                             int hpc, int groups, int n_items, int stages, unsigned int* __restrict__ sched) {
 #if defined(__CUDA_ARCH__)
   TraceScope trace_scope(trace_id);
@@ -817,6 +880,8 @@
     phase_mark(0);
     tma_prefetch_desc(&tmK);
     tma_prefetch_desc(&tmV);
+    tma_prefetch_desc(&tmKt);
+    tma_prefetch_desc(&tmVt);
     for (int s = 0; s < stages; ++s) {
       mbar_init(&full_bar[s], 1);
       mbar_init(&empty_bar[s], hpc);
@@ -842,10 +907,12 @@
         const int b = have ? item / groups : 0, grp = have ? item % groups : 0;
         const int row0 = row_base + b * t_stride;
         auto issue = [&](int ck, int s) {
-          mbar_arrive_expect_tx(&full_bar[s], static_cast<uint32_t>(stage_bytes));
+          const bool last = ck == nck - 1;
+          const int rows = last ? n_keys - ck * ATTM_CH : ATTM_CH;
+          mbar_arrive_expect_tx(&full_bar[s], static_cast<uint32_t>(2 * rows * slice_bytes));
           uint8_t* dst = ring + s * stage_bytes;
-          tma_load_3d(dst, &tmK, &full_bar[s], 0, grp * hpc, row0 + ck * ATTM_CH);
-          tma_load_3d(dst + tile_bytes, &tmV, &full_bar[s], 0, grp * hpc, row0 + ck * ATTM_CH);
+          tma_load_3d(dst, last ? &tmKt : &tmK, &full_bar[s], 0, grp * hpc, row0 + ck * ATTM_CH);
+          tma_load_3d(dst + tile_bytes, last ? &tmVt : &tmV, &full_bar[s], 0, grp * hpc, row0 + ck * ATTM_CH);
         };
         int i = 0;
         if (have && !waited && prefetch) {
@@ -1285,15 +1352,8 @@
   if (tid == 0) *dst = cand;
 }
 
-constexpr int SMPF_WARPS = 8;
-__global__ void __launch_bounds__(SMPF_WARPS * 32) sample_finalize_kernel(int trace_id, SampleArgs a, const float2* __restrict__ part,
-                                                                          int n_chunks) {
-  TraceScope trace_scope(trace_id);
-  pdl_launch_dependents();
-  pdl_wait();
+__device__ __forceinline__ int64_t finalize_row(const SampleArgs& a, const float2* __restrict__ part, int n_chunks, int r) {
   const int lane = threadIdx.x & 31;
-  const int r = blockIdx.x * SMPF_WARPS + (threadIdx.x >> 5);
-  if (r >= a.R) return;
   const int b = r / a.rows_per_b, jj = r % a.rows_per_b;
   const int slot = a.slot0 + jj;
   const float2* p = part + static_cast<size_t>(r) * n_chunks;
@@ -1326,11 +1386,50 @@
   }
 #pragma unroll
   for (int o = 16; o > 0; o >>= 1) cand = max(cand, __shfl_xor_sync(0xffffffffu, cand, o));
+  const int64_t code = static_cast<int64_t>(__float_as_int(p[cand < 0 ? 0 : cand].y));
   if (lane == 0) {
     int64_t* dst = a.dst_codes + (static_cast<size_t>(b) * a.S + a.pos) * a.dst_w +
                    (a.rows_per_b == 1 ? (a.bot_slot < 0 ? 0 : a.bot_slot) : jj);
-    *dst = static_cast<int64_t>(__float_as_int(p[cand < 0 ? 0 : cand].y));
-  }
-}
-
-}
+    *dst = code;
+  }
+  return code;
+}
+
+constexpr int SMPF_WARPS = 8;
+__global__ void __launch_bounds__(SMPF_WARPS * 32) sample_finalize_kernel(int trace_id, SampleArgs a, const float2* __restrict__ part,
+                                                                          int n_chunks) {
+  TraceScope trace_scope(trace_id);
+  pdl_launch_dependents();
+  pdl_wait();
+  const int r = blockIdx.x * SMPF_WARPS + (threadIdx.x >> 5);
+  if (r >= a.R) return;
+  finalize_row(a, part, n_chunks, r);
+}
+
+template <typename OutT>
+__global__ void __launch_bounds__(LN_THREADS)
+sample_finalize_depth_kernel(int trace_id, SampleArgs a, const float2* __restrict__ part, int n_chunks, float* __restrict__ y,
+                             const float* __restrict__ E_top_depth, const float* __restrict__ P_depth, int D,
+                             const float* __restrict__ gamma, const float* __restrict__ beta, OutT* __restrict__ h) {
+  TraceScope trace_scope(trace_id);
+  pdl_launch_dependents();
+  pdl_wait();
+  __shared__ float red[4];
+  __shared__ int64_t code;
+  const int b = blockIdx.x;
+  if (threadIdx.x < 32) {
+    const int64_t c = finalize_row(a, part, n_chunks, b);
+    if (threadIdx.x == 0) code = c;
+  }
+  __syncthreads();
+  EmbedDepthSrc src;
+  src.e = reinterpret_cast<const float4*>(E_top_depth + static_cast<size_t>(code) * D);
+#pragma unroll 1
+  for (int j = 0; j < 4; ++j) {
+    src.p = reinterpret_cast<const float4*>(P_depth + static_cast<size_t>(j) * D);
+    const size_t row = static_cast<size_t>(b) * 4 + j;
+    layernorm_row<OutT, 3>(y + row * D, gamma, beta, nullptr, h + row * D, D, nullptr, 0, 0, 0, nullptr, red, src);
+  }
+}
+
+}
diff --git a/hqtransformer_b200/engine.py b/hqtransformer_b200/engine.py
--- a/hqtransformer_b200/engine.py
+++ b/hqtransformer_b200/engine.py
@@ -263,6 +263,25 @@
     return out
 
 
+def debug_layernorm(x: torch.Tensor, gamma: torch.Tensor, beta: torch.Tensor, gamma2: torch.Tensor, beta2: torch.Tensor,
+                    add: Optional[torch.Tensor] = None, fold: Optional[torch.Tensor] = None,
+                    fold_bias: Optional[torch.Tensor] = None, fused: bool = False):
+    lib = _lib.load()
+    R, D = x.shape
+    ts = [x, gamma, beta, gamma2, beta2] + [t for t in (add, fold, fold_bias) if t is not None]
+    assert all(t.is_cuda and t.dtype == torch.float32 and t.is_contiguous() for t in ts)
+    y = torch.empty_like(x)
+    h = torch.empty(R, D, dtype=torch.bfloat16, device=x.device)
+    ptr = lambda t: None if t is None else t.data_ptr()
+    with torch.cuda.device(x.device):
+        st = torch.cuda.current_stream(x.device).cuda_stream
+        check(lib.hq_debug_layernorm(int(fused), x.data_ptr(), gamma.data_ptr(), beta.data_ptr(), ptr(add), ptr(fold),
+                                     0 if fold is None else fold.shape[0], ptr(fold_bias), gamma2.data_ptr(),
+                                     beta2.data_ptr(), y.data_ptr(), h.data_ptr(), R, D, C.c_void_p(st)),
+              None, "hq_debug_layernorm")
+    return y, h
+
+
 def debug_philox(seed: int, counter: Sequence[int]):
     lib = _lib.load()
     c = (C.c_uint32 * 4)(*counter)
diff --git a/include/hqgraft.h b/include/hqgraft.h
--- a/include/hqgraft.h
+++ b/include/hqgraft.h
@@ -129,6 +129,10 @@
 int hq_debug_attention(int prec, const void* q, const void* K, const void* V, void* out, int B, int n_heads,
                        int t_stride, int n_keys, int variant, void* stream);
 
+int hq_debug_layernorm(int fused, float* x, const float* gamma, const float* beta, const float* add, const float* fold,
+                       int n_fold, const float* fold_bias, const float* gamma2, const float* beta2, float* y, void* h,
+                       int rows, int D, void* stream);
+
 int hq_bench_attention(hq_ctx* ctx, int B, int n_keys, int iters, float* usec, void* stream);
 
 int hq_debug_attention_phases(hq_ctx* ctx, int B, int n_keys, int warm, unsigned long long* out_ns, int max_ctas,
```

Result: no change. 3539 (median of 6 runs) (+0.4%).
